# openxrlab/xrnerf

Hardware: NVIDIA B200
Metric: rays/sec (inference render, Instant-NGP lego-shaped 800x800, 65536 rays/batch) (higher is better)
Workload: dtype f16

## Files before the change

### xrnerf_b200/csrc/common.cuh

```cuda
#pragma once
#include <cuda_runtime.h>
#include <cuda_fp16.h>
#include <stdint.h>
#include <float.h>
#include "../../include/xrnerf_b200.h"

namespace xrb {

constexpr uint32_t NERF_STEPS = 1024u;
constexpr uint32_t NERF_CASCADES = 8u;
constexpr uint32_t NERF_GRIDSIZE = 128u;
constexpr uint32_t GRID_CELLS = 128u * 128u * 128u;
constexpr float NERF_MIN_OPTICAL_THICKNESS = 0.01f;
constexpr int NUM_SMS = 148;

__host__ __device__ constexpr float SQRT3() { return 1.73205080757f; }
__host__ __device__ constexpr float MIN_CONE_STEPSIZE() { return SQRT3() / NERF_STEPS; }
__host__ __device__ constexpr float MAX_CONE_STEPSIZE() { return (SQRT3() / NERF_STEPS) * (1 << (NERF_CASCADES - 1)) * NERF_STEPS / NERF_GRIDSIZE; }

void set_error(const char *msg);
int check_launch(const char *what);

#define XRB_REQUIRE(cond, msg)                                   \
    do {                                                         \
        if (!(cond)) { xrb::set_error(msg); return XRB_E_BADARG; } \
    } while (0)

struct Pcg32 {
    uint64_t state, inc;
    __host__ __device__ uint32_t next_uint() {
        uint64_t old = state;
        state = old * 0x5851f42d4c957f2dULL + inc;
        uint32_t xorshifted = (uint32_t)(((old >> 18u) ^ old) >> 27u);
        uint32_t rot = (uint32_t)(old >> 59u);
        return (xorshifted >> rot) | (xorshifted << ((~rot + 1u) & 31));
    }
    __host__ __device__ void seed(uint64_t initstate, uint64_t initseq) {
        state = 0; inc = (initseq << 1u) | 1u; next_uint(); state += initstate; next_uint();
    }
    __host__ __device__ float next_float() {
#ifdef __CUDA_ARCH__
        return __fadd_rn(__uint_as_float((next_uint() >> 9) | 0x3f800000u), -1.0f);
#else
        union { uint32_t u; float f; } x; x.u = (next_uint() >> 9) | 0x3f800000u; return x.f - 1.0f;
#endif
    }
    __host__ __device__ void advance(uint64_t delta) {
        uint64_t cur_mult = 0x5851f42d4c957f2dULL, cur_plus = inc, acc_mult = 1u, acc_plus = 0u;
        while (delta > 0) {
            if (delta & 1) { acc_mult *= cur_mult; acc_plus = acc_plus * cur_mult + cur_plus; }
            cur_plus = (cur_mult + 1) * cur_plus; cur_mult *= cur_mult; delta /= 2;
        }
        state = acc_mult * state + acc_plus;
    }
};
inline Pcg32 host_rng(uint64_t seed, int64_t n_prior_calls) {
    Pcg32 r; r.seed(seed, 1u);
    r.advance((uint64_t)n_prior_calls << 32);
    return r;
}

__host__ __device__ __forceinline__ uint32_t expand_bits(uint32_t v) {
    v = (v * 0x00010001u) & 0xFF0000FFu; v = (v * 0x00000101u) & 0x0F00F00Fu;
    v = (v * 0x00000011u) & 0xC30C30C3u; v = (v * 0x00000005u) & 0x49249249u; return v;
}
__host__ __device__ __forceinline__ uint32_t morton3D(uint32_t x, uint32_t y, uint32_t z) { return expand_bits(x) | (expand_bits(y) << 1) | (expand_bits(z) << 2); }
__host__ __device__ __forceinline__ uint32_t morton3D_invert(uint32_t x) {
    x = x & 0x49249249; x = (x | (x >> 2)) & 0xc30c30c3; x = (x | (x >> 4)) & 0x0f00f00f;
    x = (x | (x >> 8)) & 0xff0000ff; x = (x | (x >> 16)) & 0x0000ffff; return x;
}

#ifdef __CUDACC__
__device__ __forceinline__ float mul_(float a, float b) { return __fmul_rn(a, b); }
__device__ __forceinline__ float add_(float a, float b) { return __fadd_rn(a, b); }
__device__ __forceinline__ float sub_(float a, float b) { return __fsub_rn(a, b); }
__device__ __forceinline__ float div_(float a, float b) { return __fdiv_rn(a, b); }
__device__ __forceinline__ float clampf(float v, float lo, float hi) { return v < lo ? lo : (hi < v ? hi : v); }
__device__ __forceinline__ float calc_dt(float t, float cone) { return clampf(mul_(t, cone), MIN_CONE_STEPSIZE(), MAX_CONE_STEPSIZE()); }

__device__ __forceinline__ float floor_small(float p, int *ip) {
    float t = __fadd_rn(p, 12582912.0f);
    float r = __fadd_rn(t, -12582912.0f);
    int i = __float_as_int(t) - 0x4B400000;
    if (r > p) { r = __fadd_rn(r, -1.0f); i -= 1; }
    *ip = i;
    return r;
}
__device__ __forceinline__ uint32_t expand_bits7(uint32_t v) {
    v = (v | (v << 8)) & 0x0000F00Fu;
    v = (v | (v << 4)) & 0x000C30C3u;
    v = (v | (v << 2)) & 0x00249249u;
    return v;
}

__device__ __forceinline__ int frexp_exponent(float v) {
    uint32_t e = __float_as_uint(v) >> 23;
    if (e != 0) return (int)e - 126;
    if (v == 0.f) return 0;
    int r; frexpf(v, &r); return r;
}
__device__ __forceinline__ int mip_from_pos(float px, float py, float pz) {
    float m = fmaxf(fabsf(sub_(px, 0.5f)), fmaxf(fabsf(sub_(py, 0.5f)), fabsf(sub_(pz, 0.5f))));
    if (m >= 0.25f) return min((int)NERF_CASCADES - 1, (int)(__float_as_uint(m) >> 23) - 125);
    return m == 0.f ? 1 : 0;
}
__device__ __forceinline__ int mip_from_dt(float dt, float px, float py, float pz) {
    int mip = mip_from_pos(px, py, pz);
    dt = mul_(dt, (float)(2 * NERF_GRIDSIZE));
    if (dt < 1.f) return mip;
    int e = (int)(__float_as_uint(dt) >> 23) - 126;
    return min((int)NERF_CASCADES - 1, max(e, mip));
}
__device__ __forceinline__ void morton_lut_init(uint32_t *lut, int tid, int nthreads) {
    for (int v = tid; v < 128; v += nthreads) lut[v] = expand_bits7((uint32_t)v);
}
__device__ __forceinline__ uint32_t cascaded_grid_idx_at(float px, float py, float pz, uint32_t mip, const uint32_t *lut = nullptr) {
    float s = __uint_as_float((127u - mip) << 23);
    float q[3] = {px, py, pz}; uint32_t c[3];
#pragma unroll
    for (int k = 0; k < 3; ++k) {
        float v = add_(mul_(sub_(q[k], 0.5f), s), 0.5f);
        int i; floor_small(mul_(v, (float)NERF_GRIDSIZE), &i);
        c[k] = (uint32_t)min(max(i, 0), (int)NERF_GRIDSIZE - 1);
    }
    if (lut) return lut[c[0]] + (lut[c[1]] << 1) + (lut[c[2]] << 2);
    return expand_bits7(c[0]) | (expand_bits7(c[1]) << 1) | (expand_bits7(c[2]) << 2);
}
__device__ __forceinline__ bool occupied_at(float px, float py, float pz, const uint8_t *__restrict__ bitfield, uint32_t mip, const uint32_t *lut = nullptr) {
    uint32_t idx = cascaded_grid_idx_at(px, py, pz, mip, lut);
    return __ldg(bitfield + (idx >> 3) + ((GRID_CELLS * mip) >> 3)) & (1u << (idx & 7u));
}
__device__ __forceinline__ float signf_(float x) { return copysignf(1.0f, x); }
__device__ __forceinline__ float distance_to_next_voxel(const float p[3], const float d[3], const float idir[3], uint32_t res) {
    float t3[3];
#pragma unroll
    for (int k = 0; k < 3; ++k) {
        float pr = mul_((float)res, p[k]);
        int unused; float fl = floor_small(add_(add_(pr, 0.5f), mul_(0.5f, signf_(d[k]))), &unused);
        t3[k] = mul_(sub_(fl, pr), idir[k]);
    }
    float t = fminf(fminf(t3[0], t3[1]), t3[2]);
    return fmaxf(mul_(t, __uint_as_float((254u - (__float_as_uint((float)res) >> 23)) << 23)), 0.0f);
}
__device__ __forceinline__ float advance_to_next_voxel(float t, float cone, const float p[3], const float d[3], const float idir[3], uint32_t res) {
    float t_target = add_(t, distance_to_next_voxel(p, d, idir, res));
    do { t = add_(t, calc_dt(t, cone)); } while (t < t_target);
    return t;
}
__device__ __forceinline__ float aabb_ray_tmin(float lo, float hi, const float o[3], const float d[3]) {
    float tmin = div_(sub_(lo, o[0]), d[0]), tmax = div_(sub_(hi, o[0]), d[0]);
    if (tmin > tmax) { float c = tmin; tmin = tmax; tmax = c; }
    float tymin = div_(sub_(lo, o[1]), d[1]), tymax = div_(sub_(hi, o[1]), d[1]);
    if (tymin > tymax) { float c = tymin; tymin = tymax; tymax = c; }
    if (tmin > tymax || tymin > tmax) return FLT_MAX;
    if (tymin > tmin) tmin = tymin;
    if (tymax < tmax) tmax = tymax;
    float tzmin = div_(sub_(lo, o[2]), d[2]), tzmax = div_(sub_(hi, o[2]), d[2]);
    if (tzmin > tzmax) { float c = tzmin; tzmin = tzmax; tzmax = c; }
    if (tmin > tzmax || tzmin > tmax) return FLT_MAX;
    if (tzmin > tmin) tmin = tzmin;
    return tmin;
}
__device__ __forceinline__ bool aabb_contains(float lo, float hi, float x, float y, float z) {
    return x >= lo && x <= hi && y >= lo && y <= hi && z >= lo && z <= hi;
}
__device__ __forceinline__ float warp_dt(float dt) {
    const float max_stepsize = MIN_CONE_STEPSIZE() * (1 << (NERF_CASCADES - 1));
    return div_(sub_(dt, MIN_CONE_STEPSIZE()), max_stepsize - MIN_CONE_STEPSIZE());
}
__device__ __forceinline__ float unwarp_dt(float dt) {
    const float max_stepsize = MIN_CONE_STEPSIZE() * (1 << (NERF_CASCADES - 1));
    return add_(mul_(dt, max_stepsize - MIN_CONE_STEPSIZE()), MIN_CONE_STEPSIZE());
}
__device__ __forceinline__ float ray_start_t(Pcg32 rng, uint32_t i, float lo, float hi, const float o[3], const float d[3], float near_distance, float cone) {
    rng.advance((uint64_t)(i * 8u));
    float tmin = fmaxf(aabb_ray_tmin(lo, hi, o, d), near_distance);
    return add_(tmin, mul_(calc_dt(tmin, cone), rng.next_float()));
}

__device__ __forceinline__ float logistic(float x) { return 1.0f / (1.0f + expf(-x)); }
__device__ __forceinline__ float net_to_rgb(float v, int act) {
    switch (act) { case 0: return v; case 1: return v > 0.f ? v : 0.f; case 2: return logistic(v); case 3: return __expf(clampf(v, -10.f, 10.f)); }
    return 0.f;
}
__device__ __forceinline__ float net_to_density(float v, int act) {
    switch (act) { case 0: return v; case 1: return v > 0.f ? v : 0.f; case 2: return logistic(v); case 3: return __expf(v); }
    return 0.f;
}
__device__ __forceinline__ float net_to_rgb_deriv(float v, int act) {
    switch (act) { case 0: return 1.f; case 1: return v > 0.f ? 1.f : 0.f; case 2: { float s = logistic(v); return s * (1 - s); } case 3: return __expf(clampf(v, -10.f, 10.f)); }
    return 0.f;
}
__device__ __forceinline__ float net_to_density_deriv(float v, int act) {
    switch (act) { case 0: return 1.f; case 1: return v > 0.f ? 1.f : 0.f; case 2: { float s = logistic(v); return s * (1 - s); } case 3: return __expf(clampf(v, -15.f, 15.f)); }
    return 0.f;
}

__device__ __forceinline__ uint32_t warp_incl_scan_u32(uint32_t v, int lane) {
#pragma unroll
    for (int o = 1; o < 32; o <<= 1) { uint32_t n = __shfl_up_sync(0xffffffffu, v, o); if (lane >= o) v += n; }
    return v;
}
#endif

}
```

### xrnerf_b200/csrc/ngp_field.cuh

```cuda
#pragma once
#include "common.cuh"

namespace xrb {

constexpr int MAX_LEVELS = 16;
struct HashGridDev {
    uint32_t offset[MAX_LEVELS + 1];
    float scale[MAX_LEVELS];
    uint32_t res[MAX_LEVELS];
    int n_levels;
    uint32_t hashed_mask;
    uint32_t packed_mask;
    uint32_t cell_off[MAX_LEVELS];
};

inline int64_t hashgrid_build(const xrb_ngp_config *cfg, HashGridDev *g) {
    g->n_levels = cfg->n_levels; g->hashed_mask = 0;
    const float log2_pls = log2f(cfg->per_level_scale);
    uint32_t off = 0;
    for (int l = 0; l < cfg->n_levels; ++l) {
        float scale = exp2f(l * log2_pls) * (float)cfg->base_resolution - 1.0f;
        uint32_t res = (uint32_t)ceilf(scale) + 1;
        uint64_t cube = (uint64_t)res * res * res; uint32_t maxp = 0xffffffffu / 2;
        uint32_t p = cube > maxp ? maxp : (uint32_t)cube;
        p = (p + 7u) / 8u * 8u;
        uint32_t cap = 1u << cfg->log2_hashmap_size; if (p > cap) p = cap;
        if (cube > p) g->hashed_mask |= 1u << l;
        g->offset[l] = off; g->scale[l] = scale; g->res[l] = res; off += p;
    }
    g->offset[cfg->n_levels] = off;
    g->packed_mask = 0;
    for (int l = 0; l < MAX_LEVELS; ++l) g->cell_off[l] = 0;
    return (int64_t)off * cfg->n_features;
}
inline size_t cell_image_layout(HashGridDev *g, int n_packed) {
    size_t rec = 0; g->packed_mask = 0;
    for (int l = 0; l < g->n_levels && l < n_packed; ++l) {
        g->cell_off[l] = (uint32_t)rec; g->packed_mask |= 1u << l;
        rec += (size_t)g->res[l] * g->res[l] * g->res[l];
    }
    return rec * 32;
}
constexpr int MAX_PACKED_LEVELS = 13;
__host__ __device__ inline int64_t mlp_num_params(int in_w, int width, int n_hidden, int out_pad) { return (int64_t)width * in_w + (int64_t)(n_hidden - 1) * width * width + (int64_t)out_pad * width; }

inline int check_cfg(const xrb_ngp_config *cfg) {
    if (!cfg) { set_error("ngp config is null"); return XRB_E_BADARG; }
    if (cfg->n_levels != 16 || cfg->n_features != 2 || cfg->width != 64 || cfg->density_hidden < 1 || cfg->density_hidden > 4 || cfg->color_hidden < 1 || cfg->color_hidden > 4 ||
        cfg->log2_hashmap_size < 8 || cfg->log2_hashmap_size > 24 || cfg->base_resolution < 1) {
        set_error("ngp config unsupported: need n_levels=16, n_features=2, n_neurons=64, 1..4 hidden layers");
        return XRB_E_UNSUPPORTED;
    }
    return XRB_OK;
}

int table_setup(const xrb_ngp_config *cfg, const xrb_ngp_table *t, HashGridDev *g, const char *who);
struct HashGridDev;
int launch_field_ps(const xrb_ngp_config *cfg, const HashGridDev &g, const xrb_ngp_table *tab, const void *image, const float *pts, int pts_stride, const float *dirs, int dirs_stride, int n,
                    const int32_t *n_dev, float *raw, cudaStream_t s);
int launch_field(const xrb_ngp_config *cfg, const xrb_ngp_table *table, const void *dens, const void *color, const void *image, const float *pts, int pts_stride, const float *dirs,
                 int dirs_stride, int n, const int32_t *n_dev, float *out, int impl, bool density_only, cudaStream_t s);

#ifdef __CUDACC__
__device__ __forceinline__ float round_h(float x) { return __half2float(__float2half_rn(x)); }

__device__ __forceinline__ uint32_t grid_index(uint32_t x, uint32_t y, uint32_t z, uint32_t hashmap_size, uint32_t res) {
    if ((uint64_t)res * res * res > hashmap_size) {
        uint32_t h = x ^ (y * 2654435761u) ^ (z * 805459861u);
        return h & (hashmap_size - 1);
    }
    uint32_t index = x + y * res + z * res * res;
    return index >= hashmap_size ? index - hashmap_size : index;
}

struct __align__(32) Cell32 { uint32_t v[8]; };
__device__ __forceinline__ Cell32 ldg_cell(const void *p) {
    Cell32 r;
    asm volatile("ld.global.nc.v8.b32 {%0,%1,%2,%3,%4,%5,%6,%7}, [%8];"
                 : "=r"(r.v[0]), "=r"(r.v[1]), "=r"(r.v[2]), "=r"(r.v[3]), "=r"(r.v[4]), "=r"(r.v[5]), "=r"(r.v[6]), "=r"(r.v[7]) : "l"(p));
    return r;
}
__device__ __forceinline__ __half2 as_h2(uint32_t u) { return *reinterpret_cast<__half2 *>(&u); }

enum { GATHER_RUNTIME = 0, GATHER_PACKED = 1, GATHER_HASHED = 2, GATHER_DENSE = 3 };
template <int NP> __host__ __device__ constexpr int plan_mode(int l) { return NP == 0 ? GATHER_RUNTIME : (l < NP ? GATHER_PACKED : GATHER_HASHED); }
inline bool plan_valid(const HashGridDev &g, int np) {
    if (np <= 0 || np > g.n_levels) return false;
    const uint32_t all = g.n_levels >= 32 ? 0xffffffffu : ((1u << g.n_levels) - 1u), packed = (1u << np) - 1u;
    return g.packed_mask == packed && ((g.hashed_mask | packed) & all) == all;
}

__device__ __forceinline__ float2 hash_level(const __half2 *__restrict__ table, const uint8_t *__restrict__ cells, const HashGridDev &g, int l, float x, float y, float z,
                                             const int MODE = GATHER_RUNTIME) {
    const uint32_t off = g.offset[l], hs = g.offset[l + 1] - off, res = g.res[l];
    const float sc = g.scale[l];
    float px = __fmaf_rn(sc, x, 0.5f), py = __fmaf_rn(sc, y, 0.5f), pz = __fmaf_rn(sc, z, 0.5f);
    int ix_, iy_, iz_;
    float fx = floor_small(px, &ix_), fy = floor_small(py, &iy_), fz = floor_small(pz, &iz_);
    const uint32_t gx = (uint32_t)ix_, gy = (uint32_t)iy_, gz = (uint32_t)iz_;
    fx = px - fx; fy = py - fy; fz = pz - fz;
    __half2 v[8];
    const bool is_packed = MODE == GATHER_PACKED || (MODE == GATHER_RUNTIME && ((g.packed_mask >> l) & 1u));
    const bool is_hashed = MODE == GATHER_HASHED || (MODE == GATHER_RUNTIME && ((g.hashed_mask >> l) & 1u));
    if (is_packed) {
        const uint32_t rm1 = res - 1u, cx = min(gx, rm1), cy = min(gy, rm1), cz = min(gz, rm1);
        const Cell32 r = ldg_cell(cells + ((size_t)(g.cell_off[l] + cx + res * (cy + res * cz)) << 5));
#pragma unroll
        for (int c = 0; c < 8; ++c) v[c] = as_h2(r.v[c]);
    } else if (is_hashed) {
        const __half2 *tl = table + off;
        asm volatile("" : "+l"(tl));
        const uint32_t mask = hs - 1u;
        const uint32_t hy0 = gy * 2654435761u, hy1 = hy0 + 2654435761u, hz0 = gz * 805459861u, hz1 = hz0 + 805459861u;
        const uint32_t a00 = hy0 ^ hz0, a10 = hy1 ^ hz0, a01 = hy0 ^ hz1, a11 = hy1 ^ hz1, gx1 = gx + 1u;
        const uint32_t i0 = (gx ^ a00) & mask, i1 = (gx ^ a10) & mask, i2 = (gx ^ a01) & mask, i3 = (gx ^ a11) & mask;
        const uint2 w0 = __ldg(reinterpret_cast<const uint2 *>(tl + (i0 & ~1u))), w1 = __ldg(reinterpret_cast<const uint2 *>(tl + (i1 & ~1u))),
                    w2 = __ldg(reinterpret_cast<const uint2 *>(tl + (i2 & ~1u))), w3 = __ldg(reinterpret_cast<const uint2 *>(tl + (i3 & ~1u)));
        uint32_t n0 = 0, n1 = 0, n2 = 0, n3 = 0;
        const bool odd = gx & 1u;
        if (odd) {
            n0 = __ldg(reinterpret_cast<const uint32_t *>(tl + ((gx1 ^ a00) & mask))); n1 = __ldg(reinterpret_cast<const uint32_t *>(tl + ((gx1 ^ a10) & mask)));
            n2 = __ldg(reinterpret_cast<const uint32_t *>(tl + ((gx1 ^ a01) & mask))); n3 = __ldg(reinterpret_cast<const uint32_t *>(tl + ((gx1 ^ a11) & mask)));
        }
        const uint32_t e0 = (i0 & 1u) ? w0.y : w0.x, o0 = (i0 & 1u) ? w0.x : w0.y, e1 = (i1 & 1u) ? w1.y : w1.x, o1 = (i1 & 1u) ? w1.x : w1.y;
        const uint32_t e2 = (i2 & 1u) ? w2.y : w2.x, o2 = (i2 & 1u) ? w2.x : w2.y, e3 = (i3 & 1u) ? w3.y : w3.x, o3 = (i3 & 1u) ? w3.x : w3.y;
        v[0] = as_h2(e0); v[1] = as_h2(odd ? n0 : o0);
        v[2] = as_h2(e1); v[3] = as_h2(odd ? n1 : o1);
        v[4] = as_h2(e2); v[5] = as_h2(odd ? n2 : o2);
        v[6] = as_h2(e3); v[7] = as_h2(odd ? n3 : o3);
    } else {
        const __half2 *tl = table + off;
        asm volatile("" : "+l"(tl));
        const uint32_t sy = res, sz = res * res, b = gx + gy * sy + gz * sz;
#pragma unroll
        for (int c = 0; c < 8; ++c) {
            uint32_t idx = b + (c & 1) + ((c >> 1) & 1) * sy + ((c >> 2) & 1) * sz;
            idx = idx >= hs ? idx - hs : idx;
            v[c] = __ldg(tl + idx);
        }
    }
    const float ux = 1.f - fx, uy = 1.f - fy, uz = 1.f - fz;
    float2 acc = make_float2(0.f, 0.f);
#pragma unroll
    for (int c = 0; c < 8; ++c) {
        float w = ((c & 1) ? fx : ux) * ((c & 2) ? fy : uy) * ((c & 4) ? fz : uz);
        float2 f = __half22float2(v[c]);
        acc.x += w * f.x; acc.y += w * f.y;
    }
    return acc;
}

__device__ __forceinline__ void sh4(float dx01, float dy01, float dz01, float *out) {
    float x = dx01 * 2.f - 1.f, y = dy01 * 2.f - 1.f, z = dz01 * 2.f - 1.f;
    float xy = x * y, xz = x * z, yz = y * z, x2 = x * x, y2 = y * y, z2 = z * z;
    out[0] = 0.28209479177387814f;
    out[1] = -0.48860251190291987f * y;
    out[2] = 0.48860251190291987f * z;
    out[3] = -0.48860251190291987f * x;
    out[4] = 1.0925484305920792f * xy;
    out[5] = -1.0925484305920792f * yz;
    out[6] = 0.94617469575755997f * z2 - 0.31539156525251999f;
    out[7] = -1.0925484305920792f * xz;
    out[8] = 0.54627421529603959f * x2 - 0.54627421529603959f * y2;
    out[9] = 0.59004358992664352f * y * (-3.0f * x2 + y2);
    out[10] = 2.8906114426405538f * xy * z;
    out[11] = 0.45704579946446572f * y * (1.0f - 5.0f * z2);
    out[12] = 0.3731763325901154f * z * (5.0f * z2 - 3.0f);
    out[13] = 0.45704579946446572f * x * (1.0f - 5.0f * z2);
    out[14] = 1.4453057213202769f * z * (x2 - y2);
    out[15] = 0.59004358992664352f * x * (-x2 + 3.0f * y2);
}

__host__ __device__ __forceinline__ uint32_t sw128_offset(uint32_t row, uint32_t chunk16) {
    return (row >> 3) * 1024u + (row & 7u) * 128u + ((chunk16 ^ (row & 7u)) << 4);
}
struct WeightImageLayout {
    uint32_t d_in, d_hid[3], d_out, c_in, c_hid[3], c_out, total;
};
__host__ __device__ inline WeightImageLayout weight_image_layout(int density_hidden, int color_hidden) {
    WeightImageLayout L{}; uint32_t o = 0;
    L.d_in = o; o += 64 * 128;
    for (int k = 0; k < density_hidden - 1; ++k) { L.d_hid[k] = o; o += 64 * 128; }
    L.d_out = o; o += 16 * 128;
    L.c_in = o; o += 64 * 128;
    for (int k = 0; k < color_hidden - 1; ++k) { L.c_hid[k] = o; o += 64 * 128; }
    L.c_out = o; o += 16 * 128;
    L.total = o;
    return L;
}
#endif

}
```

### xrnerf_b200/csrc/ngp_fused.cu

```cuda
#include "tc_field.cuh"
#include <stdio.h>
#include <stdlib.h>

namespace xrb {

constexpr uint32_t FR_ROW_BYTES = 80;
constexpr uint32_t FR_SLOT_BYTES = 128 * FR_ROW_BYTES;
constexpr uint32_t FR_TCAP = 64;
constexpr int FR_MAX_WG = 2;

struct FusedParams {
    HashGridDev g;
    const __half2 *table; const uint8_t *cells; int np; const void *weight_image; uint32_t image_bytes; int density_hidden, color_hidden;
    const uint8_t *bitfield; const float *rays_o; const float *rays_d; int n_rays;
    float lo, hi, near_distance, cone; Pcg32 rng;
    float bg[3]; int rgb_act, dens_act;
    float *rgb_out; float *alpha_out; int32_t *n_samples_out;
    float *tscratch;
    uint32_t *sched;
    unsigned long long *dbg_out;
    int dbg;
    int field_only; const float *pts; int pts_stride; const float *dirs; int dirs_stride; int n_samples; const int32_t *n_dev; float4 *raw_out;
};

template <int FR_N_WG, int N_PROD, int N_SLOTS>
struct FusedCtl {
    uint64_t full[N_SLOTS];
    uint64_t mail[N_PROD][2];
    uint64_t mma[FR_N_WG], wbar;
    uint32_t rounds_done[N_SLOTS];
    uint32_t owner[N_SLOTS][4];
    uint32_t issued_bcast[FR_N_WG];
    uint32_t tmem_slot, ticket, closed, done, prod_done;
    uint32_t morton[128];
};
template <int FR_N_WG, int N_PROD, int N_SLOTS>
__host__ __device__ inline size_t fused_smem_bytes(uint32_t image_bytes) {
    return 1024 + image_bytes + (size_t)FR_N_WG * 16384 + (size_t)N_SLOTS * FR_SLOT_BYTES + (size_t)N_PROD * 1024 + sizeof(FusedCtl<FR_N_WG, N_PROD, N_SLOTS>) + 64;
}

__device__ __forceinline__ void spin_until_ge(volatile uint32_t *p, uint32_t v) {
    while (*p < v) __nanosleep(20);
}

template <int FR_N_WG, int N_PROD, int N_SLOTS>
__global__ void __launch_bounds__((4 * FR_N_WG + N_PROD) * 32, 3 - FR_N_WG) ngp_render_fused_kernel(const __grid_constant__ FusedParams P) {
    extern __shared__ uint8_t dyn_smem[];
    using Ctl = FusedCtl<FR_N_WG, N_PROD, N_SLOTS>;
    uint8_t *base = (uint8_t *)(((uintptr_t)dyn_smem + 1023) & ~(uintptr_t)1023);
    uint8_t *W = base, *A = W + P.image_bytes, *slots = A + (size_t)FR_N_WG * 16384, *mailbox = slots + (size_t)N_SLOTS * FR_SLOT_BYTES;
    Ctl *ctl = (Ctl *)(mailbox + (size_t)N_PROD * 1024);
    const uint32_t warp = threadIdx.x >> 5, lane = threadIdx.x & 31;
    if ((P.dbg & 8) && threadIdx.x == 0) {
        unsigned long long t0; uint32_t smid;
        asm volatile("mov.u64 %0, %%globaltimer;" : "=l"(t0)); asm volatile("mov.u32 %0, %%smid;" : "=r"(smid));
        P.dbg_out[16 * blockIdx.x] = t0; P.dbg_out[16 * blockIdx.x + 2] = smid; for (int k = 3; k < 16; ++k) P.dbg_out[16 * blockIdx.x + k] = 0;
    }

    if (threadIdx.x == 0) {
        for (int k = 0; k < N_SLOTS; ++k) { tc::mbar_init(ctl->full + k, 4); ctl->rounds_done[k] = 0; }
        for (int k = 0; k < N_PROD; ++k) { tc::mbar_init(&ctl->mail[k][0], 32); tc::mbar_init(&ctl->mail[k][1], 32); }
        for (int k = 0; k < FR_N_WG; ++k) { tc::mbar_init(ctl->mma + k, 1); ctl->issued_bcast[k] = 0; }
        tc::mbar_init(&ctl->wbar, 1);
        ctl->ticket = 0; ctl->closed = 0; ctl->done = 0; ctl->prod_done = 0;
        tc::fence_mbar_init();
        tc::mbar_expect_tx(&ctl->wbar, P.image_bytes);
        tc::tma_bulk_g2s(W, P.weight_image, P.image_bytes, &ctl->wbar);
    }
    if (warp == 1) tc::tmem_alloc<64 * FR_N_WG>(&ctl->tmem_slot);
    morton_lut_init(ctl->morton, threadIdx.x, blockDim.x);
    tc::tc_fence_before_sync();
    __syncthreads();
    tc::tc_fence_after_sync();
    const uint32_t tmem_base = ctl->tmem_slot;

    if (warp < 4 * FR_N_WG) {
        TcWarpgroup c;
        c.wg = warp >> 2; c.row = threadIdx.x & 127;
        c.A = A + (size_t)c.wg * 16384; c.W = W; c.mbar = ctl->mma + c.wg; c.tmem = tmem_base + c.wg * 64; c.phase = 0;
        const WeightImageLayout L = weight_image_layout(P.density_hidden, P.color_hidden);
        const bool timed = (P.dbg & 8) && c.wg == 0;
        tc::mbar_wait(&ctl->wbar, 0);
        long long fc[5] = {0, 0, 0, 0, 0}, ck = 0; (void)ck; (void)timed;
#ifdef XRB_FUSED_TIMERS
#define FTICK(k) do { if (timed) { long long n_ = clock64(); fc[k] += n_ - ck; ck = n_; } } while (0)
#else
#define FTICK(k) do { } while (0)
#endif
        for (uint32_t X = c.wg;; X += FR_N_WG) {
            const uint32_t s = X % N_SLOTS, r = X / N_SLOTS;
            FTICK(4);
            if (c.row == 0) {
                volatile uint32_t *tk = &ctl->ticket; volatile uint32_t *dn = &ctl->done; volatile uint32_t *cl = &ctl->closed;
                while (*cl != X) __nanosleep(20);
                uint32_t issued = 0;
                while (true) {
                    if (*tk > 4 * X) { issued = 1; break; }
                    if (*dn) { if (*tk > 4 * X) issued = 1; break; }
                    __nanosleep(20);
                }
                if (issued) {
                    while (true) {
                        uint32_t cur = *tk;
                        if (cur >= 4 * (X + 1)) { issued = 4; break; }
                        if (atomicCAS(&ctl->ticket, cur, 4 * (X + 1)) == cur) { issued = cur - 4 * X; break; }
                    }
                    for (uint32_t k = issued; k < 4; ++k) tc::mbar_arrive(ctl->full + s);
                }
                ctl->issued_bcast[c.wg] = issued;
                __threadfence_block();
                *cl = X + 1;
            }
            tc::named_bar_sync(3 + c.wg, 128);
            const uint32_t issued = *(volatile uint32_t *)&ctl->issued_bcast[c.wg];
            FTICK(0);
            if (issued == 0) { if (timed && c.row == 0) { P.dbg_out[16 * blockIdx.x + 3] = X; for (int k = 0; k < 5; ++k) P.dbg_out[16 * blockIdx.x + 4 + k] = (unsigned long long)fc[k]; } break; }
            tc::mbar_wait(ctl->full + s, r & 1);
            FTICK(1);
            const uint8_t *rowp = slots + (size_t)s * FR_SLOT_BYTES + (size_t)c.row * FR_ROW_BYTES;
            const uint4 f0 = *reinterpret_cast<const uint4 *>(rowp), f1 = *reinterpret_cast<const uint4 *>(rowp + 16), f2 = *reinterpret_cast<const uint4 *>(rowp + 32),
                        f3 = *reinterpret_cast<const uint4 *>(rowp + 48);
            const float4 dir = *reinterpret_cast<const float4 *>(rowp + 64);
            const uint32_t sub = c.row >> 5;
            const uint32_t own = ctl->owner[s][sub];
            a_store_chunk(c, 0, f0); a_store_chunk(c, 1, f1); a_store_chunk(c, 2, f2); a_store_chunk(c, 3, f3);
            tc::named_bar_sync(3 + c.wg, 128);
            if (c.row == 0) { __threadfence_block(); *(volatile uint32_t *)&ctl->rounds_done[s] = r + 1; }
            FTICK(2);
            float4 raw = make_float4(0.f, 0.f, 0.f, 0.f);
            if (!(P.dbg & 2)) {
                float dout[16];
                tc_density_from_a(c, L, P.density_hidden, dout);
                raw = tc_color_from_density(c, L, P.color_hidden, dout, dir.x, dir.y, dir.z);
            }
            FTICK(3);
            if (sub < issued) {
                *reinterpret_cast<float4 *>(mailbox + (size_t)own * 512 + (c.row & 31) * 16) = raw;
                tc::mbar_arrive(&ctl->mail[own >> 1][own & 1]);
            }
        }
    } else {
        const uint32_t pw = warp - 4 * FR_N_WG;
        float *tb = P.tscratch + ((size_t)blockIdx.x * N_PROD + pw) * 32 * FR_TCAP;
        const float diag = sub_(P.hi, P.lo);
        uint32_t n_submitted = 0;
        long long pc[7] = {0, 0, 0, 0, 0, 0, 0}, ck = 0; (void)ck;
#ifdef XRB_FUSED_TIMERS
#define PTICK(k) do { if (P.dbg & 8) { long long n_ = clock64(); pc[k] += n_ - ck; ck = n_; } } while (0)
#else
#define PTICK(k) do { } while (0)
#endif
        auto submit_chunk = [&](float x, float y, float z, float wd0, float wd1, float wd2) {
            uint32_t tk = 0;
            if (lane == 0) tk = atomicAdd(&ctl->ticket, 1u);
            tk = __shfl_sync(0xffffffffu, tk, 0);
            const uint32_t X = tk >> 2, sub = tk & 3, s = X % N_SLOTS, r = X / N_SLOTS;
            if (lane == 0) { spin_until_ge(&ctl->rounds_done[s], r); __threadfence_block(); ctl->owner[s][sub] = (pw << 1) | (n_submitted & 1); }
            __syncwarp();
            PTICK(5);
            uint8_t *rowp = slots + (size_t)s * FR_SLOT_BYTES + (size_t)(sub * 32 + lane) * FR_ROW_BYTES;
            *reinterpret_cast<float4 *>(rowp + 64) = make_float4(wd0, wd1, wd2, 0.f);
            if (P.dbg & 1) {
                for (int l = 0; l < 16; ++l) *reinterpret_cast<uint32_t *>(rowp + 4 * l) = pack_h2(x, y);
            } else if (P.np > 0) {
#pragma unroll 1
                for (int l = 0; l < P.np; ++l) {
                    const float2 f = hash_level(P.table, P.cells, P.g, l, x, y, z, GATHER_PACKED);
                    *reinterpret_cast<uint32_t *>(rowp + 4 * l) = pack_h2(f.x, f.y);
                }
#pragma unroll 1
                for (int l = P.np; l < 16; ++l) {
                    const float2 f = hash_level(P.table, P.cells, P.g, l, x, y, z, GATHER_HASHED);
                    *reinterpret_cast<uint32_t *>(rowp + 4 * l) = pack_h2(f.x, f.y);
                }
            } else {
#pragma unroll 1
                for (int l = 0; l < 16; ++l) {
                    const float2 f = hash_level(P.table, P.cells, P.g, l, x, y, z, GATHER_RUNTIME);
                    *reinterpret_cast<uint32_t *>(rowp + 4 * l) = pack_h2(f.x, f.y);
                }
            }
            __syncwarp();
            if (lane == 0) tc::mbar_arrive(ctl->full + s);
        };
        if (P.field_only) {
            int n = P.n_samples;
            if (P.n_dev) n = min(n, max(*P.n_dev, 0));
            bool pending = false, prev_valid = false; int prev_q = 0;
            const uint32_t n_pw = gridDim.x * N_PROD;
            for (uint32_t chunk = blockIdx.x * N_PROD + pw;; chunk += n_pw) {
                const bool have_chunk = (uint64_t)chunk * 32 < (uint64_t)n;
                int q = 0; bool valid = false;
                if (have_chunk) {
                    q = (int)(chunk * 32u + lane); valid = q < n;
                    float x = 0.5f, y = 0.5f, z = 0.5f, wd0 = 0.5f, wd1 = 0.5f, wd2 = 0.5f;
                    if (valid) {
                        const float *c = P.pts + (size_t)q * P.pts_stride, *d = P.dirs + (size_t)q * P.dirs_stride;
                        x = __ldg(c); y = __ldg(c + 1); z = __ldg(c + 2); wd0 = __ldg(d); wd1 = __ldg(d + 1); wd2 = __ldg(d + 2);
                    }
                    submit_chunk(x, y, z, wd0, wd1, wd2);
                }
                if (pending) {
                    const uint32_t kprev = n_submitted - 1;
                    if (lane == 0) tc::mbar_wait(&ctl->mail[pw][kprev & 1], (kprev >> 1) & 1);
                    __syncwarp();
                    const float4 raw = *reinterpret_cast<const float4 *>(mailbox + (size_t)((pw << 1) | (kprev & 1)) * 512 + lane * 16);
                    if (prev_valid) P.raw_out[prev_q] = raw;
                    pending = false;
                }
                if (!have_chunk) break;
                ++n_submitted; pending = true; prev_q = q; prev_valid = valid;
            }
        } else
        for (;;) {
            PTICK(6);
            uint32_t grp = 0;
            if (lane == 0) grp = atomicAdd(P.sched, 1u);
            grp = __shfl_sync(0xffffffffu, grp, 0);
            if ((uint64_t)grp * 32 >= (uint64_t)P.n_rays) break;
            const uint32_t ray = grp * 32 + lane;
            bool alive = ray < (uint32_t)P.n_rays;
            float t = 0.f; uint32_t nsteps = 0;
            if (alive) {
                const float o[3] = {__ldg(P.rays_o + 3 * (size_t)ray), __ldg(P.rays_o + 3 * (size_t)ray + 1), __ldg(P.rays_o + 3 * (size_t)ray + 2)};
                const float d[3] = {__ldg(P.rays_d + 3 * (size_t)ray), __ldg(P.rays_d + 3 * (size_t)ray + 1), __ldg(P.rays_d + 3 * (size_t)ray + 2)};
                t = ray_start_t(P.rng, ray, P.lo, P.hi, o, d, P.near_distance, P.cone);
            }
            float T = 1.f, ax = 0.f, ay = 0.f, az = 0.f;
            bool any_alive;
            do {
                uint32_t m = 0;
                if (alive && (P.dbg & 4)) {
                    float *tl = tb + (size_t)lane * FR_TCAP;
                    for (; m < 11; ++m) { tl[m] = t; t += 0.01f; }
                    nsteps = 11; alive = false;
                }
                if (alive) {
                    const float o[3] = {__ldg(P.rays_o + 3 * (size_t)ray), __ldg(P.rays_o + 3 * (size_t)ray + 1), __ldg(P.rays_o + 3 * (size_t)ray + 2)};
                    const float d[3] = {__ldg(P.rays_d + 3 * (size_t)ray), __ldg(P.rays_d + 3 * (size_t)ray + 1), __ldg(P.rays_d + 3 * (size_t)ray + 2)};
                    const float idir[3] = {div_(1.0f, d[0]), div_(1.0f, d[1]), div_(1.0f, d[2])};
                    float *tl = tb + (size_t)lane * FR_TCAP;
                    while (true) {
                        float p[3] = {add_(o[0], mul_(t, d[0])), add_(o[1], mul_(t, d[1])), add_(o[2], mul_(t, d[2]))};
                        if (!(aabb_contains(P.lo, P.hi, p[0], p[1], p[2]) && nsteps < NERF_STEPS)) { alive = false; break; }
                        float dt = calc_dt(t, P.cone);
                        uint32_t mip = (uint32_t)mip_from_dt(dt, p[0], p[1], p[2]);
                        if (occupied_at(p[0], p[1], p[2], P.bitfield, mip, ctl->morton)) {
                            tl[m] = t; ++m; ++nsteps; t = add_(t, dt);
                            if (m == FR_TCAP) break;
                        } else {
                            t = advance_to_next_voxel(t, P.cone, p, d, idir, NERF_GRIDSIZE >> mip);
                        }
                    }
                }
                __syncwarp();
                PTICK(0);
                any_alive = __any_sync(0xffffffffu, alive);
                const uint32_t incl = warp_incl_scan_u32(m, lane);
                const uint32_t rbase = incl - m, total = __shfl_sync(0xffffffffu, incl, 31);

                bool pending = false; uint32_t pend_key = 0; float pend_dt = 0.f;
                for (uint32_t q0 = 0; q0 < total || pending; q0 += 32) {
                    const bool have_chunk = q0 < total;
                    float dtc = 0.f; uint32_t key = 32u + lane;
                    PTICK(6);
                    if (have_chunk) {
                        const uint32_t q = q0 + lane;
                        const bool valid = q < total;
                        uint32_t j = 0;
#pragma unroll
                        for (uint32_t step = 16; step >= 1; step >>= 1) {
                            const uint32_t cand = j + step;
                            const uint32_t b = __shfl_sync(0xffffffffu, rbase, cand & 31);
                            if (cand < 32 && b <= q) j = cand;
                        }
                        const uint32_t bj = __shfl_sync(0xffffffffu, rbase, j);
                        float x = 0.5f, y = 0.5f, z = 0.5f, wd0 = 0.5f, wd1 = 0.5f, wd2 = 0.5f;
                        if (valid) {
                            const float tt = *(volatile float *)(tb + (size_t)j * FR_TCAP + (q - bj));
                            const size_t rj = (size_t)grp * 32 + j;
                            const float oj0 = __ldg(P.rays_o + 3 * rj), oj1 = __ldg(P.rays_o + 3 * rj + 1), oj2 = __ldg(P.rays_o + 3 * rj + 2);
                            const float dj0 = __ldg(P.rays_d + 3 * rj), dj1 = __ldg(P.rays_d + 3 * rj + 1), dj2 = __ldg(P.rays_d + 3 * rj + 2);
                            x = div_(sub_(add_(oj0, mul_(tt, dj0)), P.lo), diag); y = div_(sub_(add_(oj1, mul_(tt, dj1)), P.lo), diag); z = div_(sub_(add_(oj2, mul_(tt, dj2)), P.lo), diag);
                            wd0 = mul_(add_(dj0, 1.0f), 0.5f); wd1 = mul_(add_(dj1, 1.0f), 0.5f); wd2 = mul_(add_(dj2, 1.0f), 0.5f);
                            dtc = unwarp_dt(warp_dt(calc_dt(tt, P.cone)));
                            key = j;
                        }
#ifdef XRB_FUSED_TIMERS
                        if (P.dbg & 8) { if (__float_as_uint(x + y + z + dtc) == 0x7fc12345u) pc[6] += 1; }
#endif
                        PTICK(1);
                        submit_chunk(x, y, z, wd0, wd1, wd2);
                        PTICK(2);
                    }
                    if (pending) {
                        const uint32_t kprev = n_submitted - 1;
                        if (lane == 0) tc::mbar_wait(&ctl->mail[pw][kprev & 1], (kprev >> 1) & 1);
                        __syncwarp();
                        PTICK(3);
                        const float4 raw = *reinterpret_cast<const float4 *>(mailbox + (size_t)((pw << 1) | (kprev & 1)) * 512 + lane * 16);
                        float alpha = 0.f, sx = 0.f, sy = 0.f, sz = 0.f;
                        if (pend_key < 32) {
                            const float density = net_to_density(raw.w, P.dens_act);
                            alpha = 1.f - __expf(-density * pend_dt);
                            sx = alpha * net_to_rgb(raw.x, P.rgb_act); sy = alpha * net_to_rgb(raw.y, P.rgb_act); sz = alpha * net_to_rgb(raw.z, P.rgb_act);
                        }
                        float pr = 1.f - alpha;
                        const uint32_t prev_key = __shfl_up_sync(0xffffffffu, pend_key, 1);
                        const uint32_t heads = __ballot_sync(0xffffffffu, lane == 0 || pend_key != prev_key);
                        const int seg_start = 31 - __clz(heads & (0xffffffffu >> (31 - lane)));
#pragma unroll
                        for (int off = 1; off < 32; off <<= 1) {
                            const float np = __shfl_up_sync(0xffffffffu, pr, off), nx = __shfl_up_sync(0xffffffffu, sx, off), ny = __shfl_up_sync(0xffffffffu, sy, off),
                                        nz = __shfl_up_sync(0xffffffffu, sz, off);
                            if ((int)lane - off >= seg_start) { sx = nx + np * sx; sy = ny + np * sy; sz = nz + np * sz; pr = np * pr; }
                        }
                        const uint32_t pq0 = q0 - 32;
                        const uint32_t lo_q = max(rbase, pq0), hi_q = min(rbase + m, q0);
                        const uint32_t tail = (hi_q - 1 - pq0) & 31;
                        const float gp = __shfl_sync(0xffffffffu, pr, tail), gx = __shfl_sync(0xffffffffu, sx, tail), gy = __shfl_sync(0xffffffffu, sy, tail),
                                    gz = __shfl_sync(0xffffffffu, sz, tail);
                        if (hi_q > lo_q) { ax += T * gx; ay += T * gy; az += T * gz; T *= gp; }
                        pending = false;
                        PTICK(4);
                    }
                    if (have_chunk) { ++n_submitted; pending = true; pend_key = key; pend_dt = dtc; }
                }
            } while (any_alive);
            if (ray < (uint32_t)P.n_rays) {
                P.rgb_out[3 * (size_t)ray] = ax + T * P.bg[0]; P.rgb_out[3 * (size_t)ray + 1] = ay + T * P.bg[1]; P.rgb_out[3 * (size_t)ray + 2] = az + T * P.bg[2];
                P.alpha_out[ray] = 1.f - T;
                if (P.n_samples_out) P.n_samples_out[ray] = (int32_t)nsteps;
            }
        }
        if ((P.dbg & 8) && lane == 0) { for (int k = 0; k < 7; ++k) atomicAdd(P.dbg_out + 16 * blockIdx.x + 9 + k, (unsigned long long)pc[k]); }
        if (lane == 0) {
            __threadfence_block();
            if (atomicAdd(&ctl->prod_done, 1u) == N_PROD - 1) *(volatile uint32_t *)&ctl->done = 1u;
        }
    }
    tc::tc_fence_before_sync();
    __syncthreads();
    if (warp == 1) tc::tmem_dealloc<64 * FR_N_WG>(tmem_base);
    if ((P.dbg & 8) && threadIdx.x == 0) { unsigned long long t1; asm volatile("mov.u64 %0, %%globaltimer;" : "=l"(t1)); P.dbg_out[16 * blockIdx.x + 1] = t1; }
    if (threadIdx.x == 0 && !P.field_only) {
        __threadfence();
        if (atomicAdd(P.sched + 1, 1u) == gridDim.x - 1) { P.sched[0] = 0; P.sched[1] = 0; __threadfence(); }
    }
}

constexpr int FUSED_MAX_PROD_PER_SM = 24;
static int fused_variant() { static int v = -1; if (v < 0) { const char *e = getenv("XRB_FUSED_VARIANT"); v = e ? atoi(e) : 0; if (v != 0 && v != 1) v = 0; } return v; }

int launch_field_ps(const xrb_ngp_config *cfg, const HashGridDev &g, const xrb_ngp_table *tab, const void *image, const float *pts, int pts_stride, const float *dirs, int dirs_stride, int n,
                    const int32_t *n_dev, float *raw, cudaStream_t s) {
    FusedParams P{};
    P.g = g;
    P.table = (const __half2 *)tab->table_fp16; P.cells = (const uint8_t *)tab->cell_image; P.np = plan_valid(P.g, tab->n_packed_levels) ? tab->n_packed_levels : 0;
    P.weight_image = image; P.image_bytes = weight_image_layout(cfg->density_hidden, cfg->color_hidden).total;
    P.density_hidden = cfg->density_hidden; P.color_hidden = cfg->color_hidden;
    P.field_only = 1; P.pts = pts; P.pts_stride = pts_stride; P.dirs = dirs; P.dirs_stride = dirs_stride; P.n_samples = n; P.n_dev = n_dev; P.raw_out = (float4 *)raw;
    { static const int dbg = getenv("XRB_FUSED_DBG") ? atoi(getenv("XRB_FUSED_DBG")) : 0; P.dbg = dbg & 3; }
    int dev = 0, sms = NUM_SMS; cudaGetDevice(&dev); cudaDeviceGetAttribute(&sms, cudaDevAttrMultiProcessorCount, dev);
    auto k = ngp_render_fused_kernel<2, 16, 5>;
    const size_t smem = fused_smem_bytes<2, 16, 5>(P.image_bytes);
    cudaFuncSetAttribute(k, cudaFuncAttributeMaxDynamicSharedMemorySize, (int)smem);
    const int64_t n_chunks = ((int64_t)n + 31) / 32;
    int grid = sms; if (n_chunks < (int64_t)grid * 16) grid = (int)((n_chunks + 15) / 16); if (grid < 1) grid = 1;
    k<<<grid, (4 * 2 + 16) * 32, smem, s>>>(P);
    return check_launch("ngp_mlp_forward (producer/consumer)");
}

}

using namespace xrb;

extern "C" {

size_t xrb_ngp_render_fused_workspace(void) {
    int dev = 0, sms = NUM_SMS; cudaGetDevice(&dev); if (cudaDeviceGetAttribute(&sms, cudaDevAttrMultiProcessorCount, dev) != cudaSuccess) { cudaGetLastError(); sms = NUM_SMS; }
    return 256 + (size_t)sms * FUSED_MAX_PROD_PER_SM * 32 * FR_TCAP * sizeof(float) + (size_t)sms * 2 * 128;
}

int xrb_ngp_render_fused(const xrb_ngp_config *cfg, const xrb_ngp_table *table, const void *weight_image, const uint8_t *bitfield, const float *rays_o, const float *rays_d, int n_rays,
                         float aabb0, float aabb1, float near_distance, float cone_angle, uint64_t seed, int64_t n_prior_calls, const float *bg3_host, int rgb_act, int dens_act,
                         float *rgb_out, float *alpha_out, int32_t *n_samples_out, void *workspace, void *stream) {
    int e = check_cfg(cfg); if (e) return e;
    XRB_REQUIRE(n_rays >= 0, "ngp_render_fused: bad size");
    if (n_rays == 0) return XRB_OK;
    XRB_REQUIRE(table && weight_image && bitfield && rays_o && rays_d && bg3_host && rgb_out && alpha_out && workspace, "ngp_render_fused: null pointer");
    XRB_REQUIRE(((uintptr_t)workspace & 255) == 0 && ((uintptr_t)weight_image & 15) == 0, "ngp_render_fused: workspace must be 256-byte aligned, weight image 16-byte aligned");
    FusedParams P;
    e = table_setup(cfg, table, &P.g, "ngp_render_fused"); if (e) return e;
    P.table = (const __half2 *)table->table_fp16; P.cells = (const uint8_t *)table->cell_image; P.np = plan_valid(P.g, table->n_packed_levels) ? table->n_packed_levels : 0;
    P.weight_image = weight_image; P.image_bytes = weight_image_layout(cfg->density_hidden, cfg->color_hidden).total;
    P.density_hidden = cfg->density_hidden; P.color_hidden = cfg->color_hidden;
    P.bitfield = bitfield; P.rays_o = rays_o; P.rays_d = rays_d; P.n_rays = n_rays;
    P.lo = aabb0; P.hi = aabb1; P.near_distance = near_distance; P.cone = cone_angle; P.rng = host_rng(seed, n_prior_calls);
    P.bg[0] = bg3_host[0]; P.bg[1] = bg3_host[1]; P.bg[2] = bg3_host[2]; P.rgb_act = rgb_act; P.dens_act = dens_act;
    P.rgb_out = rgb_out; P.alpha_out = alpha_out; P.n_samples_out = n_samples_out;
    { static const int dbg = getenv("XRB_FUSED_DBG") ? atoi(getenv("XRB_FUSED_DBG")) : 0; P.dbg = dbg; }
    int dev = 0, sms = NUM_SMS; cudaGetDevice(&dev); cudaDeviceGetAttribute(&sms, cudaDevAttrMultiProcessorCount, dev);
    P.sched = (uint32_t *)workspace; P.tscratch = (float *)((uint8_t *)workspace + 256);
    P.dbg_out = (unsigned long long *)((uint8_t *)workspace + 256 + (size_t)sms * FUSED_MAX_PROD_PER_SM * 32 * FR_TCAP * sizeof(float));
    const int64_t n_groups = ((int64_t)n_rays + 31) / 32;
    P.field_only = 0; P.pts = nullptr; P.dirs = nullptr; P.pts_stride = P.dirs_stride = 0; P.n_samples = 0; P.n_dev = nullptr; P.raw_out = nullptr;
#define XRB_LAUNCH_FUSED(NWG, NP, NS)                                                                                                                  \
    do {                                                                                                                                               \
        auto k = ngp_render_fused_kernel<NWG, NP, NS>;                                                                                                 \
        const size_t smem = fused_smem_bytes<NWG, NP, NS>(P.image_bytes);                                                                              \
        cudaFuncSetAttribute(k, cudaFuncAttributeMaxDynamicSharedMemorySize, (int)smem);    \
        int grid = sms * (3 - NWG); if (n_groups < grid) grid = (int)n_groups;                                                                         \
        k<<<grid, (4 * NWG + NP) * 32, smem, (cudaStream_t)stream>>>(P);                                                                               \
    } while (0)
    if (fused_variant() == 1) XRB_LAUNCH_FUSED(1, 8, 3); else XRB_LAUNCH_FUSED(2, 16, 5);
#undef XRB_LAUNCH_FUSED
    return check_launch("ngp_render_fused");
}

}
```

### xrnerf_b200/csrc/ngp_mlp.cu

```cuda
#include "tc_field.cuh"
#include <stdio.h>
#include <stdlib.h>

namespace xrb {

__global__ void __launch_bounds__(256) cast_f32_to_f16_kernel(const float *__restrict__ src, __half *__restrict__ dst, int64_t n) {
    int64_t i = ((int64_t)blockIdx.x * blockDim.x + threadIdx.x) * 4;
    const int64_t stride = (int64_t)gridDim.x * blockDim.x * 4;
    for (; i + 3 < n; i += stride) {
        float4 v = *reinterpret_cast<const float4 *>(src + i);
        __half2 a = __floats2half2_rn(v.x, v.y), b = __floats2half2_rn(v.z, v.w);
        uint2 o; o.x = *reinterpret_cast<uint32_t *>(&a); o.y = *reinterpret_cast<uint32_t *>(&b);
        *reinterpret_cast<uint2 *>(dst + i) = o;
    }
    if (blockIdx.x == 0 && threadIdx.x < 4) { int64_t t = (n & ~(int64_t)3) + threadIdx.x; if (t < n) dst[t] = __float2half_rn(src[t]); }
}

__global__ void pack_weights_kernel(const float *__restrict__ dens, const float *__restrict__ color, uint8_t *__restrict__ image, int density_hidden, int color_hidden) {
    const WeightImageLayout L = weight_image_layout(density_hidden, color_hidden);
    const int n_mats = density_hidden + 1 + color_hidden + 1;
    for (int m = blockIdx.x; m < n_mats; m += gridDim.x) {
        const bool is_color = m > density_hidden;
        const int li = is_color ? m - (density_hidden + 1) : m;
        const int n_hidden = is_color ? color_hidden : density_hidden;
        const float *params = is_color ? color : dens;
        const int K = li == 0 ? 32 : 64, N = li == n_hidden ? 16 : 64;
        size_t poff = 0;
        for (int q = 0; q < li; ++q) poff += (size_t)64 * (q == 0 ? 32 : 64);
        const float *Wm = params + poff;
        uint32_t ioff = is_color ? (li == 0 ? L.c_in : (li == n_hidden ? L.c_out : L.c_hid[li - 1])) : (li == 0 ? L.d_in : (li == n_hidden ? L.d_out : L.d_hid[li - 1]));
        for (int t = threadIdx.x; t < N * 8; t += blockDim.x) {
            int row = t >> 3, chunk = t & 7;
            __half h[8];
#pragma unroll
            for (int e = 0; e < 8; ++e) { int k = chunk * 8 + e; h[e] = k < K ? __float2half_rn(Wm[(size_t)row * K + k]) : __float2half_rn(0.f); }
            *reinterpret_cast<uint4 *>(image + ioff + sw128_offset(row, chunk)) = *reinterpret_cast<uint4 *>(h);
        }
    }
}

__global__ void __launch_bounds__(256) cell_image_build_kernel(HashGridDev g, const __half2 *__restrict__ table, uint32_t *__restrict__ image, int n_packed, uint64_t n_words) {
    for (uint64_t t = (uint64_t)blockIdx.x * blockDim.x + threadIdx.x; t < n_words; t += (uint64_t)gridDim.x * blockDim.x) {
        const uint32_t rec = (uint32_t)(t >> 3), c = (uint32_t)t & 7u;
        int l = 0;
#pragma unroll
        for (int k = 1; k < MAX_PACKED_LEVELS; ++k) if (k < n_packed && rec >= g.cell_off[k]) l = k;
        const uint32_t res = g.res[l], cell = rec - g.cell_off[l];
        const uint32_t gx = cell % res, gy = (cell / res) % res, gz = cell / (res * res);
        const uint32_t hs = g.offset[l + 1] - g.offset[l];
        const uint32_t idx = grid_index(gx + (c & 1u), gy + ((c >> 1) & 1u), gz + ((c >> 2) & 1u), hs, res);
        image[t] = reinterpret_cast<const uint32_t *>(table)[g.offset[l] + idx];
    }
}

__global__ void __launch_bounds__(256) hashgrid_forward_kernel(HashGridDev g, const __half2 *__restrict__ table, const uint8_t *__restrict__ cells, const float *__restrict__ x,
                                                               int x_stride, int n, __half2 *__restrict__ enc) {
    int64_t t = (int64_t)blockIdx.x * blockDim.x + threadIdx.x;
    int64_t i = t >> 4; int l = (int)(t & 15);
    if (i >= n) return;
    const float *p = x + (size_t)i * x_stride;
    float2 f = hash_level(table, cells, g, l, p[0], p[1], p[2]);
    enc[(size_t)i * 16 + l] = __floats2half2_rn(f.x, f.y);
}
__global__ void __launch_bounds__(256) sh4_forward_kernel(const float *__restrict__ dirs, int stride, int n, __half *__restrict__ out) {
    int i = blockIdx.x * blockDim.x + threadIdx.x;
    if (i >= n) return;
    const float *d = dirs + (size_t)i * stride;
    float s[16]; sh4(d[0], d[1], d[2], s);
    __half h[16];
#pragma unroll
    for (int k = 0; k < 16; ++k) h[k] = __float2half_rn(s[k]);
    uint4 *o = reinterpret_cast<uint4 *>(out + (size_t)i * 16);
    o[0] = reinterpret_cast<uint4 *>(h)[0]; o[1] = reinterpret_cast<uint4 *>(h)[1];
}

template <int IN, int OUT, bool RELU>
__device__ __forceinline__ void simt_layer(const __half *__restrict__ W, const float *x, float *y) {
#pragma unroll
    for (int o = 0; o < OUT; ++o) {
        float s = 0.f;
        const __half2 *w2 = reinterpret_cast<const __half2 *>(W + (size_t)o * IN);
#pragma unroll
        for (int k = 0; k < IN / 2; ++k) { float2 w = __half22float2(w2[k]); s = fmaf(w.x, x[2 * k], s); s = fmaf(w.y, x[2 * k + 1], s); }
        y[o] = round_h(RELU ? fmaxf(s, 0.f) : s);
    }
}
__device__ __forceinline__ void simt_net(const __half *__restrict__ P, int n_hidden, const float *x32, float *out16) {
    float a[64], b[64];
    simt_layer<32, 64, true>(P, x32, a); P += 64 * 32;
    for (int h = 0; h < n_hidden - 1; ++h) {
        simt_layer<64, 64, true>(P, a, b); P += 64 * 64;
#pragma unroll
        for (int k = 0; k < 64; ++k) a[k] = b[k];
    }
    simt_layer<64, 16, false>(P, a, out16);
}

template <bool DENSITY_ONLY>
__global__ void __launch_bounds__(128) ngp_field_simt_kernel(HashGridDev g, const __half2 *__restrict__ table, const uint8_t *__restrict__ cells, const __half *__restrict__ dens_p, const __half *__restrict__ color_p,
                                                             int density_hidden, int color_hidden, const float *__restrict__ pts, int pts_stride, const float *__restrict__ dirs,
                                                             int dirs_stride, int n, const int32_t *__restrict__ n_dev, float *__restrict__ out) {
    extern __shared__ __half s_w[];
    if (n_dev) n = min(n, max(*n_dev, 0));
    const int nd = (int)mlp_num_params(32, 64, density_hidden, 16), nc = DENSITY_ONLY ? 0 : (int)mlp_num_params(32, 64, color_hidden, 16);
    for (int k = threadIdx.x; k < nd; k += blockDim.x) s_w[k] = dens_p[k];
    for (int k = threadIdx.x; k < nc; k += blockDim.x) s_w[nd + k] = color_p[k];
    __syncthreads();
    for (int i = blockIdx.x * blockDim.x + threadIdx.x; i < n; i += gridDim.x * blockDim.x) {
        const float *p = pts + (size_t)i * pts_stride;
        float enc[32];
#pragma unroll
        for (int l = 0; l < 16; ++l) { float2 f = hash_level(table, cells, g, l, p[0], p[1], p[2]); enc[2 * l] = round_h(f.x); enc[2 * l + 1] = round_h(f.y); }
        float dout[16];
        simt_net(s_w, density_hidden, enc, dout);
        if (DENSITY_ONLY) { out[i] = dout[0]; continue; }
        const float *d = dirs + (size_t)i * dirs_stride;
        float cin[32], sh[16];
        sh4(d[0], d[1], d[2], sh);
#pragma unroll
        for (int k = 0; k < 15; ++k) cin[k] = dout[k + 1];
#pragma unroll
        for (int k = 0; k < 16; ++k) cin[15 + k] = round_h(sh[k]);
        cin[31] = 1.0f;
        float cout[16];
        simt_net(s_w + nd, color_hidden, cin, cout);
        reinterpret_cast<float4 *>(out)[i] = make_float4(cout[0], cout[1], cout[2], dout[0]);
    }
}

__global__ void __launch_bounds__(128) mlp_forward_simt_kernel(const __half *__restrict__ params, const __half *__restrict__ x, int n, int n_hidden, __half *__restrict__ y) {
    extern __shared__ __half s_w[];
    const int np = (int)mlp_num_params(32, 64, n_hidden, 16);
    for (int k = threadIdx.x; k < np; k += blockDim.x) s_w[k] = params[k];
    __syncthreads();
    for (int i = blockIdx.x * blockDim.x + threadIdx.x; i < n; i += gridDim.x * blockDim.x) {
        float xin[32], out[16];
#pragma unroll
        for (int k = 0; k < 32; ++k) xin[k] = __half2float(x[(size_t)i * 32 + k]);
        simt_net(s_w, n_hidden, xin, out);
#pragma unroll
        for (int k = 0; k < 16; ++k) y[(size_t)i * 16 + k] = __float2half_rn(out[k]);
    }
}

template <bool DENSITY_ONLY, int NWG, int MAXREG, int NP>
__global__ void __launch_bounds__(128 * NWG, NWG == 2 ? 2 : 1) __maxnreg__(MAXREG)
ngp_field_tc_kernel(HashGridDev g, const __half2 *__restrict__ table, const uint8_t *__restrict__ cells, const void *__restrict__ weight_image, uint32_t image_bytes, int density_hidden,
                    int color_hidden, const float *__restrict__ pts, int pts_stride, const float *__restrict__ dirs, int dirs_stride, int n, const int32_t *__restrict__ n_dev,
                    float *__restrict__ out, int dbg) {
    extern __shared__ uint8_t dyn_smem[];
    if (n_dev) n = min(n, max(*n_dev, 0));
    constexpr uint32_t TMEM_COLS = NWG <= 2 ? 128 : (NWG <= 4 ? 256 : 512);
    TcWarpgroup c = tc_cta_setup<NWG, TMEM_COLS>(dyn_smem, weight_image, image_bytes);
    const uint32_t tmem_base = c.tmem - c.wg * 64;
    const WeightImageLayout L = weight_image_layout(density_hidden, color_hidden);
    const int n_tiles = (n + 127) / 128;
    if (!(dbg & 7)) {
        const int stride = gridDim.x * NWG;
        int tile = blockIdx.x * NWG + c.wg;
        if (tile < n_tiles) {
            uint32_t e[16];
            float dx = 0.5f, dy = 0.5f, dz = 0.5f;
            {
                const int i = tile * 128 + c.row;
                float x = 0.5f, y = 0.5f, z = 0.5f;
                if (i < n) {
                    const float *p = pts + (size_t)i * pts_stride; x = p[0]; y = p[1]; z = p[2];
                    if (!DENSITY_ONLY) { const float *d = dirs + (size_t)i * dirs_stride; dx = d[0]; dy = d[1]; dz = d[2]; }
                }
                tc_gather_levels<NP, 0, 16>(table, cells, g, x, y, z, e);
            }
            for (; tile < n_tiles; tile += stride) {
                const int i = tile * 128 + c.row, in = i + stride * 128;
                const bool has_next = tile + stride < n_tiles;
                float xn = 0.5f, yn = 0.5f, zn = 0.5f, dxn = 0.5f, dyn = 0.5f, dzn = 0.5f;
                if (has_next && in < n) {
                    const float *p = pts + (size_t)in * pts_stride; xn = p[0]; yn = p[1]; zn = p[2];
                    if (!DENSITY_ONLY) { const float *d = dirs + (size_t)in * dirs_stride; dxn = d[0]; dyn = d[1]; dzn = d[2]; }
                }
                uint32_t en[16];
                const float4 raw = tc_field_gather_ahead<NP, DENSITY_ONLY>(c, L, density_hidden, color_hidden, table, cells, g, e, dx, dy, dz, has_next, xn, yn, zn, en);
                if (i < n) { if (DENSITY_ONLY) out[i] = raw.x; else reinterpret_cast<float4 *>(out)[i] = raw; }
#pragma unroll
                for (int k = 0; k < 16; ++k) e[k] = en[k];
                dx = dxn; dy = dyn; dz = dzn;
            }
        }
        tc_cta_teardown<TMEM_COLS>(tmem_base);
        return;
    }
    for (int tile = blockIdx.x * NWG + c.wg; tile < n_tiles; tile += gridDim.x * NWG) {
        const int i = tile * 128 + c.row;
        const bool valid = i < n;
        float x = 0.5f, y = 0.5f, z = 0.5f, dx = 0.5f, dy = 0.5f, dz = 0.5f;
        if (valid) {
            const float *p = pts + (size_t)i * pts_stride; x = p[0]; y = p[1]; z = p[2];
            if (!DENSITY_ONLY) { const float *d = dirs + (size_t)i * dirs_stride; dx = d[0]; dy = d[1]; dz = d[2]; }
        }
        float dout[16];
        if (dbg & 1) {
#pragma unroll
            for (int q = 0; q < 4; ++q) a_store_chunk(c, q, make_uint4(pack_h2(x, y), pack_h2(z, x), pack_h2(y, z), pack_h2(x, z)));
            if (dbg & 2) { for (int k = 0; k < 16; ++k) dout[k] = x; } else tc_density_from_a(c, L, density_hidden, dout);
        } else if (dbg & 2) {
            float acc = 0.f;
#pragma unroll
            for (int l = 0; l < 16; ++l) { float2 f = hash_level(table, cells, g, l, x, y, z, plan_mode<NP>(l)); acc += f.x + f.y; }
            for (int k = 0; k < 16; ++k) dout[k] = acc;
        } else {
            tc_density<NP>(c, L, density_hidden, table, cells, g, x, y, z, dout);
        }
        if (DENSITY_ONLY) {
            if (valid) out[i] = dout[0];
        } else {
            float4 raw = (dbg & 2) ? make_float4(dout[0], dout[1], dout[2], dout[3]) : tc_color_from_density(c, L, color_hidden, dout, dx, dy, dz);
            if (valid) reinterpret_cast<float4 *>(out)[i] = raw;
        }
    }
    tc_cta_teardown<TMEM_COLS>(tmem_base);
}

static int persistent_grid(const void *kernel, int block, size_t smem, int work_ctas, int min_per_sm = 1) {
    int per_sm = 1;
    cudaError_t oe = cudaOccupancyMaxActiveBlocksPerMultiprocessor(&per_sm, kernel, block, smem);
    if (getenv("XRB_DEBUG")) fprintf(stderr, "[xrb] occupancy query: err=%d per_sm=%d block=%d smem=%zu\n", (int)oe, per_sm, block, smem);
    if (oe != cudaSuccess) cudaGetLastError();
    if (per_sm < min_per_sm) per_sm = min_per_sm;
    int dev = 0, sms = NUM_SMS; cudaGetDevice(&dev); cudaDeviceGetAttribute(&sms, cudaDevAttrMultiProcessorCount, dev);
    int g = sms * per_sm;
    return work_ctas < g ? (work_ctas > 0 ? work_ctas : 1) : g;
}

}

using namespace xrb;

extern "C" {

int64_t xrb_tcnn_hashgrid_num_params(const xrb_ngp_config *cfg) { if (check_cfg(cfg)) return -1; HashGridDev g; return hashgrid_build(cfg, &g); }
int64_t xrb_tcnn_density_num_params(const xrb_ngp_config *cfg) { if (check_cfg(cfg)) return -1; return mlp_num_params(32, 64, cfg->density_hidden, 16); }
int64_t xrb_tcnn_color_num_params(const xrb_ngp_config *cfg) { if (check_cfg(cfg)) return -1; return mlp_num_params(32, 64, cfg->color_hidden, 16); }
int xrb_tcnn_hashgrid_layout(const xrb_ngp_config *cfg, uint32_t *offsets_host, float *scales_host, uint32_t *res_host) {
    int e = check_cfg(cfg); if (e) return e;
    HashGridDev g; hashgrid_build(cfg, &g);
    for (int l = 0; l <= cfg->n_levels; ++l) if (offsets_host) offsets_host[l] = g.offset[l];
    for (int l = 0; l < cfg->n_levels; ++l) { if (scales_host) scales_host[l] = g.scale[l]; if (res_host) res_host[l] = g.res[l]; }
    return XRB_OK;
}

int xrb_tcnn_cast_params(const float *src, void *dst_fp16, int64_t n, void *stream) {
    XRB_REQUIRE(n >= 0, "cast_params: negative size");
    if (n == 0) return XRB_OK;
    XRB_REQUIRE(src && dst_fp16, "cast_params: null pointer");
    XRB_REQUIRE(((uintptr_t)src & 15) == 0 && ((uintptr_t)dst_fp16 & 7) == 0, "cast_params: misaligned");
    int64_t blocks = (n / 4 + 255) / 256; if (blocks > NUM_SMS * 16) blocks = NUM_SMS * 16; if (blocks < 1) blocks = 1;
    cast_f32_to_f16_kernel<<<(int)blocks, 256, 0, (cudaStream_t)stream>>>(src, (__half *)dst_fp16, n);
    return check_launch("cast_params");
}

size_t xrb_ngp_weight_image_bytes(const xrb_ngp_config *cfg) { if (check_cfg(cfg)) return 0; return weight_image_layout(cfg->density_hidden, cfg->color_hidden).total; }

int xrb_ngp_pack_weights(const xrb_ngp_config *cfg, const float *density_params, const float *color_params, void *image, void *stream) {
    int e = check_cfg(cfg); if (e) return e;
    XRB_REQUIRE(density_params && color_params && image, "pack_weights: null pointer");
    XRB_REQUIRE(((uintptr_t)image & 15) == 0, "pack_weights: image must be 16-byte aligned");
    pack_weights_kernel<<<cfg->density_hidden + cfg->color_hidden + 2, 256, 0, (cudaStream_t)stream>>>(density_params, color_params, (uint8_t *)image, cfg->density_hidden, cfg->color_hidden);
    return check_launch("pack_weights");
}

size_t xrb_ngp_cell_image_bytes(const xrb_ngp_config *cfg, int n_packed_levels) {
    if (check_cfg(cfg) || n_packed_levels <= 0) return 0;
    if (n_packed_levels > MAX_PACKED_LEVELS) n_packed_levels = MAX_PACKED_LEVELS;
    HashGridDev g; hashgrid_build(cfg, &g);
    return cell_image_layout(&g, n_packed_levels);
}

int xrb_ngp_build_cell_image(const xrb_ngp_config *cfg, const void *table_fp16, int n_packed_levels, void *cell_image, void *stream) {
    int e = check_cfg(cfg); if (e) return e;
    XRB_REQUIRE(n_packed_levels >= 0 && n_packed_levels <= MAX_PACKED_LEVELS, "build_cell_image: n_packed_levels must be 0..13");
    if (n_packed_levels == 0) return XRB_OK;
    XRB_REQUIRE(table_fp16 && cell_image, "build_cell_image: null pointer");
    XRB_REQUIRE(((uintptr_t)cell_image & 31) == 0 && ((uintptr_t)table_fp16 & 15) == 0, "build_cell_image: cell image must be 32-byte, table 16-byte aligned");
    HashGridDev g; hashgrid_build(cfg, &g);
    const uint64_t n_words = cell_image_layout(&g, n_packed_levels) / 4;
    uint64_t blocks = (n_words + 255) / 256; if (blocks > (uint64_t)NUM_SMS * 32) blocks = (uint64_t)NUM_SMS * 32;
    cell_image_build_kernel<<<(unsigned)blocks, 256, 0, (cudaStream_t)stream>>>(g, (const __half2 *)table_fp16, (uint32_t *)cell_image, n_packed_levels, n_words);
    return check_launch("build_cell_image");
}

}
namespace xrb {
int table_setup(const xrb_ngp_config *cfg, const xrb_ngp_table *t, HashGridDev *g, const char *who) {
    if (!t || !t->table_fp16) { set_error("null hash table"); return XRB_E_BADARG; }
    if (((uintptr_t)t->table_fp16 & 15) != 0) { set_error("hash table must be 16-byte aligned"); return XRB_E_BADARG; }
    hashgrid_build(cfg, g);
    if (t->n_packed_levels < 0 || t->n_packed_levels > MAX_PACKED_LEVELS) { set_error("n_packed_levels must be 0..13"); return XRB_E_BADARG; }
    if (t->n_packed_levels > 0) {
        if (!t->cell_image || ((uintptr_t)t->cell_image & 31) != 0) { set_error("cell image missing or not 32-byte aligned"); return XRB_E_BADARG; }
        cell_image_layout(g, t->n_packed_levels);
    }
    (void)who;
    return XRB_OK;
}
}
extern "C" {

int xrb_tcnn_hashgrid_forward(const xrb_ngp_config *cfg, const xrb_ngp_table *table, const float *x, int x_stride, int n, void *enc_fp16, void *stream) {
    int e = check_cfg(cfg); if (e) return e;
    XRB_REQUIRE(n >= 0 && x_stride >= 3, "hashgrid_forward: bad size");
    if (n == 0) return XRB_OK;
    XRB_REQUIRE(table && x && enc_fp16, "hashgrid_forward: null pointer");
    HashGridDev g; e = table_setup(cfg, table, &g, "hashgrid_forward"); if (e) return e;
    int64_t threads = (int64_t)n * 16;
    hashgrid_forward_kernel<<<(unsigned)((threads + 255) / 256), 256, 0, (cudaStream_t)stream>>>(g, (const __half2 *)table->table_fp16, (const uint8_t *)table->cell_image, x, x_stride, n,
                                                                                                 (__half2 *)enc_fp16);
    return check_launch("hashgrid_forward");
}

int xrb_tcnn_sh4_forward(const float *dirs, int dir_stride, int n, void *out_fp16, void *stream) {
    XRB_REQUIRE(n >= 0 && dir_stride >= 3, "sh4_forward: bad size");
    if (n == 0) return XRB_OK;
    XRB_REQUIRE(dirs && out_fp16, "sh4_forward: null pointer");
    sh4_forward_kernel<<<(n + 255) / 256, 256, 0, (cudaStream_t)stream>>>(dirs, dir_stride, n, (__half *)out_fp16);
    return check_launch("sh4_forward");
}

int xrb_tcnn_mlp_forward(const void *params_fp16, const void *x_fp16, int n, int in_w, int width, int n_hidden, void *y_fp16, void *stream) {
    XRB_REQUIRE(n >= 0, "mlp_forward: negative size");
    if (in_w != 32 || width != 64 || n_hidden < 1 || n_hidden > 4) { set_error("mlp_forward: only in=32 (padded), width=64, 1..4 hidden layers"); return XRB_E_UNSUPPORTED; }
    if (n == 0) return XRB_OK;
    XRB_REQUIRE(params_fp16 && x_fp16 && y_fp16, "mlp_forward: null pointer");
    size_t smem = mlp_num_params(32, 64, n_hidden, 16) * sizeof(__half);
    if (smem > 48 * 1024) cudaFuncSetAttribute(mlp_forward_simt_kernel, cudaFuncAttributeMaxDynamicSharedMemorySize, (int)smem);
    int grid = persistent_grid((const void *)mlp_forward_simt_kernel, 128, smem, (n + 127) / 128);
    mlp_forward_simt_kernel<<<grid, 128, smem, (cudaStream_t)stream>>>((const __half *)params_fp16, (const __half *)x_fp16, n, n_hidden, (__half *)y_fp16);
    return check_launch("mlp_forward");
}

}
namespace xrb {
int launch_field(const xrb_ngp_config *cfg, const xrb_ngp_table *tab, const void *dens, const void *color, const void *image, const float *pts, int pts_stride, const float *dirs,
                 int dirs_stride, int n, const int32_t *n_dev, float *out, int impl, bool density_only, cudaStream_t s) {
    HashGridDev g; int e = table_setup(cfg, tab, &g, "field"); if (e) return e;
    const void *table = tab->table_fp16; const uint8_t *cells = (const uint8_t *)tab->cell_image;
    if (impl == 0) {
        size_t smem = (mlp_num_params(32, 64, cfg->density_hidden, 16) + (density_only ? 0 : mlp_num_params(32, 64, cfg->color_hidden, 16))) * sizeof(__half);
        const void *k = density_only ? (const void *)ngp_field_simt_kernel<true> : (const void *)ngp_field_simt_kernel<false>;
        if (smem > 48 * 1024) cudaFuncSetAttribute(k, cudaFuncAttributeMaxDynamicSharedMemorySize, (int)smem);
        int grid = persistent_grid(k, 128, smem, (n + 127) / 128);
        if (density_only)
            ngp_field_simt_kernel<true><<<grid, 128, smem, s>>>(g, (const __half2 *)table, cells, (const __half *)dens, (const __half *)color, cfg->density_hidden, cfg->color_hidden, pts, pts_stride,
                                                                dirs, dirs_stride, n, n_dev, out);
        else
            ngp_field_simt_kernel<false><<<grid, 128, smem, s>>>(g, (const __half2 *)table, cells, (const __half *)dens, (const __half *)color, cfg->density_hidden, cfg->color_hidden, pts, pts_stride,
                                                                 dirs, dirs_stride, n, n_dev, out);
    } else {
        uint32_t image_bytes = weight_image_layout(cfg->density_hidden, cfg->color_hidden).total;
        static const int env_shape = getenv("XRB_TC_SHAPE") ? atoi(getenv("XRB_TC_SHAPE")) : -1;
        const int shape = env_shape >= 0 ? env_shape : 0;
        static const int dbg = getenv("XRB_FIELD_DBG") ? atoi(getenv("XRB_FIELD_DBG")) : 0;
        if (shape == 4 && !density_only && (((uintptr_t)out) & 15) == 0) return launch_field_ps(cfg, g, tab, image, pts, pts_stride, dirs, dirs_stride, n, n_dev, out, s);
        const int npl = tab->n_packed_levels;
        const int np = (plan_valid(g, npl) && (npl == 6 || npl == 7)) ? npl : 0;
        int n_tiles = (n + 127) / 128;
#define XRB_LAUNCH_TC(D, NWG, R, NP)                                                                                                                \
    do {                                                                                                                                            \
        auto k = ngp_field_tc_kernel<D, NWG, R, NP>;                                                                                                \
        const size_t smem = tc_cta_smem_bytes<NWG>(image_bytes);                                                                                    \
        cudaFuncSetAttribute(k, cudaFuncAttributeMaxDynamicSharedMemorySize, (int)smem);                                                            \
        int grid = persistent_grid((const void *)k, 128 * NWG, smem, (n_tiles + NWG - 1) / NWG, NWG == 2 ? 2 : 1);                                  \
        k<<<grid, 128 * NWG, smem, s>>>(g, (const __half2 *)table, cells, image, image_bytes, cfg->density_hidden, cfg->color_hidden, pts, pts_stride, dirs, dirs_stride, n, n_dev, out, dbg); \
    } while (0)
#define XRB_LAUNCH_TC_NP(D, NWG, R)                                                                                                                 \
    do {                                                                                                                                            \
        if (np == 6) XRB_LAUNCH_TC(D, NWG, R, 6); else if (np == 7) XRB_LAUNCH_TC(D, NWG, R, 7); else XRB_LAUNCH_TC(D, NWG, R, 0);                   \
    } while (0)
#define XRB_LAUNCH_TC_SHAPE(D)                                                                                                                      \
    do {                                                                                                                                            \
        if (shape == 1) XRB_LAUNCH_TC_NP(D, 2, 128); else if (shape == 2) XRB_LAUNCH_TC_NP(D, 6, 80); else if (shape == 3) XRB_LAUNCH_TC_NP(D, 8, 64); else XRB_LAUNCH_TC_NP(D, 2, 96); \
    } while (0)
        if (density_only) XRB_LAUNCH_TC_SHAPE(true); else XRB_LAUNCH_TC_SHAPE(false);
#undef XRB_LAUNCH_TC_SHAPE
#undef XRB_LAUNCH_TC_NP
#undef XRB_LAUNCH_TC
    }
    return check_launch(density_only ? "ngp_density_forward" : "ngp_mlp_forward");
}
}
extern "C" {

int xrb_ngp_mlp_forward(const xrb_ngp_config *cfg, const xrb_ngp_table *table, const void *density_fp16, const void *color_fp16, const void *weight_image, const float *pts, int pts_stride,
                        const float *dirs, int dirs_stride, int n, const int32_t *n_rows_dev, float *raw, int impl, void *stream) {
    int e = check_cfg(cfg); if (e) return e;
    XRB_REQUIRE(n >= 0 && pts_stride >= 3 && dirs_stride >= 3, "ngp_mlp_forward: bad size");
    if (n == 0) return XRB_OK;
    XRB_REQUIRE(table && pts && dirs && raw, "ngp_mlp_forward: null pointer");
    XRB_REQUIRE(((uintptr_t)raw & 15) == 0, "ngp_mlp_forward: raw must be 16-byte aligned");
    XRB_REQUIRE(impl == 0 ? (density_fp16 && color_fp16) : (weight_image != nullptr), "ngp_mlp_forward: missing weights for the requested impl");
    return launch_field(cfg, table, density_fp16, color_fp16, weight_image, pts, pts_stride, dirs, dirs_stride, n, n_rows_dev, raw, impl, false, (cudaStream_t)stream);
}

int xrb_ngp_density_forward(const xrb_ngp_config *cfg, const xrb_ngp_table *table, const void *density_fp16, const void *weight_image, const float *pts, int pts_stride, int n, float *density,
                            int impl, void *stream) {
    int e = check_cfg(cfg); if (e) return e;
    XRB_REQUIRE(n >= 0 && pts_stride >= 3, "ngp_density_forward: bad size");
    if (n == 0) return XRB_OK;
    XRB_REQUIRE(table && pts && density, "ngp_density_forward: null pointer");
    XRB_REQUIRE(impl == 0 ? (density_fp16 != nullptr) : (weight_image != nullptr), "ngp_density_forward: missing weights for the requested impl");
    return launch_field(cfg, table, density_fp16, nullptr, weight_image, pts, pts_stride, nullptr, 3, n, nullptr, density, impl, true, (cudaStream_t)stream);
}

}
```

### xrnerf_b200/csrc/ngp_render.cu

```cuda
#include "ngp_field.cuh"

extern "C" {

size_t xrb_ngp_render_workspace(int n_rays, int max_samples) {
    size_t a = (xrb_rm_rays_sampler_workspace(n_rays) + 255) & ~(size_t)255;
    return a + (size_t)max_samples * (7 + 4) * sizeof(float) + (size_t)n_rays * sizeof(int32_t) + 256;
}

int xrb_ngp_render(const xrb_ngp_config *cfg, const xrb_ngp_table *table, const void *weight_image, const uint8_t *bitfield, const float *rays_o, const float *rays_d, int n_rays,
                   int max_samples, float aabb0, float aabb1, float near_distance, float cone_angle, uint64_t seed, int64_t n_prior_calls, const float *bg3_host, int rgb_act,
                   int dens_act, float *rgb_out, float *alpha_out, int32_t *numsteps, int32_t *counters, void *workspace, void *ev_before_field, void *ev_after_field, void *stream) {
    int e = xrb::check_cfg(cfg); if (e) return e;
    XRB_REQUIRE(n_rays >= 0 && max_samples > 0, "ngp_render: bad size");
    if (n_rays == 0) return XRB_OK;
    XRB_REQUIRE(table && weight_image && bitfield && rays_o && rays_d && bg3_host && rgb_out && alpha_out && numsteps && counters && workspace, "ngp_render: null pointer");
    cudaStream_t s = (cudaStream_t)stream;
    uint8_t *ws = (uint8_t *)workspace;
    size_t a = (xrb_rm_rays_sampler_workspace(n_rays) + 255) & ~(size_t)255;
    float *coords = (float *)(ws + a);
    float *raw = coords + (size_t)max_samples * 7;
    int32_t *rays_index = (int32_t *)(raw + (size_t)max_samples * 4);
    cudaMemsetAsync(counters, 0, 2 * sizeof(int32_t), s);
    e = xrb_rm_rays_sampler(rays_o, rays_d, bitfield, nullptr, nullptr, nullptr, n_rays, max_samples, aabb0, aabb1, near_distance, cone_angle, seed, n_prior_calls, coords, rays_index,
                            numsteps, counters, ws, stream);
    if (e) return e;
    if (ev_before_field) cudaEventRecord((cudaEvent_t)ev_before_field, s);
    e = xrb::launch_field(cfg, table, nullptr, nullptr, weight_image, coords, 7, coords + 4, 7, max_samples, counters + 1, raw, 1, false, s);
    if (ev_after_field) cudaEventRecord((cudaEvent_t)ev_after_field, s);
    if (e) return e;
    return xrb_rm_calc_rgb_inference(raw, coords, numsteps, bg3_host, n_rays, rgb_act, dens_act, rgb_out, alpha_out, stream);
}

}
```

### xrnerf_b200/csrc/raymarch.cu

```cuda
#include "common.cuh"
#include <stdio.h>
#include <string.h>
#include <stdlib.h>

namespace xrb {

static thread_local char g_err[256] = "";
void set_error(const char *msg) { strncpy(g_err, msg, sizeof(g_err) - 1); g_err[sizeof(g_err) - 1] = 0; }
int check_launch(const char *what) {
    cudaError_t e = cudaGetLastError();
    if (e != cudaSuccess) { snprintf(g_err, sizeof g_err, "%s: %s", what, cudaGetErrorString(e)); return (int)e; }
    return XRB_OK;
}

constexpr uint32_t TCAP = 64;
constexpr uint32_t OVF_CAP = NERF_STEPS - TCAP;
struct OvfPool { uint32_t *counter; float *area; uint32_t n_chunks; int32_t *chunk_of; };

template <bool EMIT>
__device__ __forceinline__ uint32_t march_ray(const float o[3], const float d[3], float lo, float hi, float startt, float cone,
                                              const uint8_t *__restrict__ bitfield, uint32_t limit, float *__restrict__ coords, float *__restrict__ tbuf = nullptr,
                                              const uint32_t *lut = nullptr, const OvfPool *pool = nullptr, uint32_t ray = 0) {
    const float idir[3] = {div_(1.0f, d[0]), div_(1.0f, d[1]), div_(1.0f, d[2])};
    float wdir[3], diag = sub_(hi, lo);
    if (EMIT) { wdir[0] = mul_(add_(d[0], 1.0f), 0.5f); wdir[1] = mul_(add_(d[1], 1.0f), 0.5f); wdir[2] = mul_(add_(d[2], 1.0f), 0.5f); }
    uint32_t j = 0; float t = startt;
    float *ovf = nullptr;
    while (true) {
        float p[3] = {add_(o[0], mul_(t, d[0])), add_(o[1], mul_(t, d[1])), add_(o[2], mul_(t, d[2]))};
        if (!(aabb_contains(lo, hi, p[0], p[1], p[2]) && j < limit)) break;
        float dt = calc_dt(t, cone);
        uint32_t mip = (uint32_t)mip_from_dt(dt, p[0], p[1], p[2]);
        if (occupied_at(p[0], p[1], p[2], bitfield, mip, lut)) {
            if (EMIT) {
                float *c = coords + 7 * (size_t)j;
                c[0] = div_(sub_(p[0], lo), diag); c[1] = div_(sub_(p[1], lo), diag); c[2] = div_(sub_(p[2], lo), diag);
                c[3] = warp_dt(dt);
                c[4] = wdir[0]; c[5] = wdir[1]; c[6] = wdir[2];
            } else if (tbuf) {
                if (j < TCAP) tbuf[j] = t;
                else if (pool) {
                    if (j == TCAP) {
                        const uint32_t c = atomicAdd(pool->counter, 1u);
                        const bool got = c < pool->n_chunks;
                        pool->chunk_of[ray] = got ? (int32_t)c : -1;
                        ovf = got ? pool->area + (size_t)c * OVF_CAP : nullptr;
                    }
                    if (ovf) ovf[j - TCAP] = t;
                }
            }
            ++j; t = add_(t, dt);
        } else {
            t = advance_to_next_voxel(t, cone, p, d, idir, NERF_GRIDSIZE >> mip);
        }
    }
    return j;
}

constexpr int MARCH_BLOCK = 128;
static inline int warp_grid(int n_rays) { size_t b = ((size_t)n_rays * 32 + 255) / 256, cap = (size_t)NUM_SMS * 8; return (int)(b < cap ? (b ? b : 1) : cap); }
constexpr int MAX_LANE_STRIDE = 4;
constexpr int MARCH_RAYS_PER_BLOCK_MIN = MARCH_BLOCK / MAX_LANE_STRIDE;
static int lane_stride() { static int v = -1; if (v < 0) { const char *e = getenv("XRB_MARCH_LANE_STRIDE"); v = e ? atoi(e) : 1; if (v != 1 && v != 2 && v != 4) v = 1; } return v; }

struct MarchWs {
    uint32_t *local_excl;
    float *startt;
    uint32_t *block_sum;
    uint32_t *misc;
    float *tbuf;
    int32_t *chunk_of;
    float *ovf;
    uint32_t n_chunks;
};
__host__ __device__ inline uint32_t march_n_chunks(int n) { uint32_t c = (uint32_t)n / 8u; return c < 64u ? 64u : c; }
__host__ __device__ inline size_t march_ws_bytes(int n) {
    size_t nb = (size_t)(n + MARCH_RAYS_PER_BLOCK_MIN - 1) / MARCH_RAYS_PER_BLOCK_MIN;
    return sizeof(uint32_t) * ((size_t)n * 3 + nb + 16 + (size_t)n * TCAP + (size_t)march_n_chunks(n) * OVF_CAP);
}
inline MarchWs march_ws(void *ws, int n) {
    size_t nb = (size_t)(n + MARCH_RAYS_PER_BLOCK_MIN - 1) / MARCH_RAYS_PER_BLOCK_MIN;
    MarchWs w; w.local_excl = (uint32_t *)ws; w.startt = (float *)(w.local_excl + n); w.block_sum = (uint32_t *)(w.startt + n); w.misc = w.block_sum + nb; w.tbuf = (float *)(w.misc + 16);
    w.chunk_of = (int32_t *)(w.tbuf + (size_t)n * TCAP); w.ovf = (float *)(w.chunk_of + n); w.n_chunks = march_n_chunks(n);
    return w;
}

__device__ __forceinline__ uint32_t block_excl_scan(uint32_t v, uint32_t *total) {
    __shared__ uint32_t warp_tot[MARCH_BLOCK / 32];
    int lane = threadIdx.x & 31, w = threadIdx.x >> 5;
    uint32_t incl = warp_incl_scan_u32(v, lane);
    if (lane == 31) warp_tot[w] = incl;
    __syncthreads();
    uint32_t off = 0, tot = 0;
#pragma unroll
    for (int k = 0; k < MARCH_BLOCK / 32; ++k) { uint32_t s = warp_tot[k]; if (k < w) off += s; tot += s; }
    *total = tot;
    return off + incl - v;
}

template <int LANE_STRIDE>
__global__ void __launch_bounds__(MARCH_BLOCK) march_count_kernel(int n_rays, const float *__restrict__ rays_o, const float *__restrict__ rays_d,
                                                                  const uint8_t *__restrict__ bitfield, float lo, float hi, float near_distance, float cone,
                                                                  Pcg32 rng, uint32_t *__restrict__ local_excl, float *__restrict__ startt_out,
                                                                  uint32_t *__restrict__ block_sum, int32_t *__restrict__ numsteps, float *__restrict__ tbuf, OvfPool pool) {
    constexpr int MARCH_RAYS_PER_BLOCK = MARCH_BLOCK / LANE_STRIDE;
    __shared__ uint32_t lut[128];
    morton_lut_init(lut, threadIdx.x, MARCH_BLOCK);
    __syncthreads();
    const bool owner = (threadIdx.x % LANE_STRIDE) == 0;
    uint32_t i = blockIdx.x * MARCH_RAYS_PER_BLOCK + threadIdx.x / LANE_STRIDE;
    uint32_t n = 0;
    if (owner && i < (uint32_t)n_rays) {
        float o[3] = {rays_o[3 * (size_t)i], rays_o[3 * (size_t)i + 1], rays_o[3 * (size_t)i + 2]};
        float d[3] = {rays_d[3 * (size_t)i], rays_d[3 * (size_t)i + 1], rays_d[3 * (size_t)i + 2]};
        float st = ray_start_t(rng, i, lo, hi, o, d, near_distance, cone);
        startt_out[i] = st;
        n = march_ray<false>(o, d, lo, hi, st, cone, bitfield, NERF_STEPS, nullptr, tbuf ? tbuf + (size_t)i * TCAP : nullptr, lut, tbuf ? &pool : nullptr, i);
        numsteps[2 * (size_t)i] = (int32_t)n;
    }
    uint32_t tot;
    uint32_t ex = block_excl_scan(n, &tot);
    if (owner && i < (uint32_t)n_rays) local_excl[i] = ex;
    if (threadIdx.x == 0) block_sum[blockIdx.x] = tot;
}

__global__ void __launch_bounds__(1024) march_scan_kernel(int n_blocks, uint32_t *__restrict__ block_sum, uint32_t *__restrict__ misc, int32_t *__restrict__ counters) {
    __shared__ uint32_t warp_tot[32];
    __shared__ uint32_t carry_s;
    int lane = threadIdx.x & 31, w = threadIdx.x >> 5;
    if (threadIdx.x == 0) carry_s = 0;
    __syncthreads();
    for (int b0 = 0; b0 < n_blocks; b0 += 1024) {
        int b = b0 + threadIdx.x;
        uint32_t v = b < n_blocks ? block_sum[b] : 0u;
        uint32_t incl = warp_incl_scan_u32(v, lane);
        if (lane == 31) warp_tot[w] = incl;
        __syncthreads();
        uint32_t off = 0, tot = 0;
        for (int k = 0; k < 32; ++k) { uint32_t s = warp_tot[k]; if (k < w) off += s; tot += s; }
        uint32_t carry = carry_s;
        if (b < n_blocks) block_sum[b] = carry + off + incl - v;
        __syncthreads();
        if (threadIdx.x == 0) carry_s = carry + tot;
        __syncthreads();
    }
    if (threadIdx.x == 0) {
        uint32_t base0 = counters ? (uint32_t)counters[1] : 0u, ray0 = counters ? (uint32_t)counters[0] : 0u;
        misc[0] = base0; misc[1] = ray0; misc[2] = carry_s;
        if (counters) counters[1] = (int32_t)(base0 + carry_s);
    }
}

__global__ void __launch_bounds__(256) march_emit_kernel(int n_rays, const float *__restrict__ rays_o, const float *__restrict__ rays_d, const uint8_t *__restrict__ bitfield, float lo,
                                                         float hi, float cone, uint32_t max_samples, const uint32_t *__restrict__ local_excl, const float *__restrict__ startt,
                                                         const uint32_t *__restrict__ block_off, const uint32_t *__restrict__ misc, const float *__restrict__ tbuf,
                                                         const int32_t *__restrict__ chunk_of, const float *__restrict__ ovf, float *__restrict__ coords_out, int32_t *__restrict__ rays_index, int32_t *__restrict__ numsteps,
                                                         int32_t *__restrict__ counters, int rays_per_scan_block) {
    const int lane = threadIdx.x & 31;
    const uint32_t n_warps = (gridDim.x * 256) >> 5;
    uint32_t ok_count = 0;
    for (uint32_t i = (blockIdx.x * 256 + threadIdx.x) >> 5; i < (uint32_t)n_rays; i += n_warps) {
        uint32_t n = (uint32_t)numsteps[2 * (size_t)i];
        uint32_t base = misc[0] + block_off[i / rays_per_scan_block] + local_excl[i];
        __syncwarp();
        if (base + n > max_samples) {
            if (lane == 0) { numsteps[2 * (size_t)i] = 0; numsteps[2 * (size_t)i + 1] = (int32_t)base; }
        } else {
            ok_count += 1;
            if (lane == 0) {
                numsteps[2 * (size_t)i + 1] = (int32_t)base;
                rays_index[i] = n == 0 ? -1 : (int32_t)(misc[1] + i);
            }
            if (n > 0) {
                const float o[3] = {rays_o[3 * (size_t)i], rays_o[3 * (size_t)i + 1], rays_o[3 * (size_t)i + 2]};
                const float d[3] = {rays_d[3 * (size_t)i], rays_d[3 * (size_t)i + 1], rays_d[3 * (size_t)i + 2]};
                const float diag = sub_(hi, lo);
                const float w0 = mul_(add_(d[0], 1.0f), 0.5f), w1 = mul_(add_(d[1], 1.0f), 0.5f), w2 = mul_(add_(d[2], 1.0f), 0.5f);
                const int32_t chunk = n > TCAP ? chunk_of[i] : -1;
                const float *tl = tbuf + (size_t)i * TCAP, *to = chunk >= 0 ? ovf + (size_t)chunk * OVF_CAP : nullptr;
                const uint32_t n_par = n <= TCAP ? n : (to ? n : TCAP - 1);
                for (uint32_t j = lane; j < n_par; j += 32) {
                    float t = j < TCAP ? tl[j] : to[j - TCAP];
                    float *c = coords_out + 7 * (size_t)(base + j);
                    c[0] = div_(sub_(add_(o[0], mul_(t, d[0])), lo), diag); c[1] = div_(sub_(add_(o[1], mul_(t, d[1])), lo), diag); c[2] = div_(sub_(add_(o[2], mul_(t, d[2])), lo), diag);
                    c[3] = warp_dt(calc_dt(t, cone));
                    c[4] = w0; c[5] = w1; c[6] = w2;
                }
                if (n_par < n && lane == 0) march_ray<true>(o, d, lo, hi, tl[TCAP - 1], cone, bitfield, n - (TCAP - 1), coords_out + 7 * (size_t)(base + TCAP - 1));
            }
        }
    }
    if (lane == 0 && ok_count && counters) atomicAdd((unsigned int *)counters, ok_count);
}

__global__ void __launch_bounds__(MARCH_BLOCK) compact_count_kernel(int n_rays, const int32_t *__restrict__ numsteps, uint32_t *__restrict__ local_excl,
                                                                    uint32_t *__restrict__ block_sum) {
    uint32_t i = blockIdx.x * MARCH_BLOCK + threadIdx.x;
    uint32_t n = i < (uint32_t)n_rays ? (uint32_t)numsteps[2 * (size_t)i] : 0u;
    uint32_t tot, ex = block_excl_scan(n, &tot);
    if (i < (uint32_t)n_rays) local_excl[i] = ex;
    if (threadIdx.x == 0) block_sum[blockIdx.x] = tot;
}
__global__ void __launch_bounds__(256) compact_copy_kernel(int n_rays, uint32_t max_compacted, const float *__restrict__ coords_in, const int32_t *__restrict__ numsteps,
                                                           const uint32_t *__restrict__ local_excl, const uint32_t *__restrict__ block_off, const uint32_t *__restrict__ misc,
                                                           float *__restrict__ coords_out, int32_t *__restrict__ numsteps_c, int32_t *__restrict__ ray_counter) {
    int lane = threadIdx.x & 31;
    uint32_t ray = (blockIdx.x * 256 + threadIdx.x) >> 5;
    if (ray >= (uint32_t)n_rays) return;
    uint32_t n = (uint32_t)numsteps[2 * (size_t)ray], base = (uint32_t)numsteps[2 * (size_t)ray + 1];
    uint32_t cbase = misc[0] + block_off[ray / MARCH_BLOCK] + local_excl[ray];
    uint32_t nc = min(max_compacted - min(max_compacted, cbase), n);
    if (lane == 0) { numsteps_c[2 * (size_t)ray] = (int32_t)nc; numsteps_c[2 * (size_t)ray + 1] = (int32_t)cbase; if (nc) atomicAdd((unsigned int *)ray_counter, 1u); }
    const float *src = coords_in + 7 * (size_t)base; float *dst = coords_out + 7 * (size_t)cbase;
    for (uint32_t k = lane; k < nc * 7; k += 32) dst[k] = src[k];
}

__global__ void __launch_bounds__(256) count_trained_kernel(int n_rays, const int32_t *__restrict__ numsteps, const int32_t *__restrict__ numsteps_c, unsigned long long *__restrict__ accum) {
    unsigned int local = 0;
    for (int i = blockIdx.x * blockDim.x + threadIdx.x; i < n_rays; i += gridDim.x * blockDim.x) local += numsteps_c[2 * (size_t)i] == numsteps[2 * (size_t)i] ? 1u : 0u;
#pragma unroll
    for (int o = 16; o > 0; o >>= 1) local += __shfl_xor_sync(0xffffffffu, local, o);
    if ((threadIdx.x & 31) == 0 && local) atomicAdd(accum, (unsigned long long)local);
}

__device__ __forceinline__ float warp_excl_prod(float v, int lane, float *incl_out) {
    float incl = v;
#pragma unroll
    for (int o = 1; o < 32; o <<= 1) { float n = __shfl_up_sync(0xffffffffu, incl, o); if (lane >= o) incl *= n; }
    float ex = __shfl_up_sync(0xffffffffu, incl, 1);
    *incl_out = incl;
    return lane == 0 ? 1.f : ex;
}
__device__ __forceinline__ float warp_incl_sum(float v, int lane) {
#pragma unroll
    for (int o = 1; o < 32; o <<= 1) { float n = __shfl_up_sync(0xffffffffu, v, o); if (lane >= o) v += n; }
    return v;
}
__device__ __forceinline__ float warp_sum(float v) {
#pragma unroll
    for (int o = 16; o > 0; o >>= 1) v += __shfl_xor_sync(0xffffffffu, v, o);
    return v;
}

template <int MODE>
__global__ void __launch_bounds__(256) composite_fwd_kernel(int n_rays, const float4 *__restrict__ raw, const float *__restrict__ coords, const int32_t *__restrict__ numsteps,
                                                            const int32_t *__restrict__ numsteps_c, const float *__restrict__ bg, float3 bg_global, int rgb_act, int dens_act,
                                                            float *__restrict__ rgb_out, float *__restrict__ alpha_out) {
    int lane = threadIdx.x & 31;
    const uint32_t n_warps = (gridDim.x * 256) >> 5;
    for (uint32_t ray = (blockIdx.x * 256 + threadIdx.x) >> 5; ray < (uint32_t)n_rays; ray += n_warps) {
    const int32_t *ns = MODE == 0 ? numsteps_c : numsteps;
    uint32_t n = (uint32_t)ns[2 * (size_t)ray], base = (uint32_t)ns[2 * (size_t)ray + 1];
    float3 b = MODE == 0 ? make_float3(bg[3 * (size_t)ray], bg[3 * (size_t)ray + 1], bg[3 * (size_t)ray + 2]) : bg_global;
    if (n == 0) {
        if (lane == 0) { rgb_out[3 * (size_t)ray] = b.x; rgb_out[3 * (size_t)ray + 1] = b.y; rgb_out[3 * (size_t)ray + 2] = b.z; if (MODE == 1) alpha_out[ray] = 0.f; }
        continue;
    }
    float T = 1.f, ax = 0.f, ay = 0.f, az = 0.f;
    for (uint32_t k0 = 0; k0 < n; k0 += 32) {
        uint32_t k = k0 + lane; bool valid = k < n;
        float alpha = 0.f, cx = 0.f, cy = 0.f, cz = 0.f;
        if (valid) {
            float4 r = __ldg(raw + base + k);
            float dt = unwarp_dt(__ldg(coords + 7 * (size_t)(base + k) + 3));
            float density = net_to_density(r.w, dens_act);
            alpha = 1.f - __expf(-density * dt);
            cx = net_to_rgb(r.x, rgb_act); cy = net_to_rgb(r.y, rgb_act); cz = net_to_rgb(r.z, rgb_act);
        }
        float incl, ex = warp_excl_prod(1.f - alpha, lane, &incl);
        float w = alpha * (T * ex);
        ax += w * cx; ay += w * cy; az += w * cz;
        T *= __shfl_sync(0xffffffffu, incl, 31);
    }
    ax = warp_sum(ax); ay = warp_sum(ay); az = warp_sum(az);
    if (lane == 0) {
        bool add_bg = MODE == 1 ? true : (n == (uint32_t)numsteps[2 * (size_t)ray]);
        if (add_bg) { ax += T * b.x; ay += T * b.y; az += T * b.z; }
        rgb_out[3 * (size_t)ray] = ax; rgb_out[3 * (size_t)ray + 1] = ay; rgb_out[3 * (size_t)ray + 2] = az;
        if (MODE == 1) alpha_out[ray] = 1.f - T;
    }
    }
}

__global__ void __launch_bounds__(256) composite_bwd_kernel(int n_rays, const float4 *__restrict__ raw, const float *__restrict__ coords, const int32_t *__restrict__ numsteps_c,
                                                            const float *__restrict__ grad_rgb, const float *__restrict__ rgb_final, const float *__restrict__ grid_mean,
                                                            int rgb_act, int dens_act, float4 *__restrict__ dl_draw) {
    int lane = threadIdx.x & 31;
    const uint32_t n_warps = (gridDim.x * 256) >> 5;
    for (uint32_t ray = (blockIdx.x * 256 + threadIdx.x) >> 5; ray < (uint32_t)n_rays; ray += n_warps) {
    uint32_t n = (uint32_t)numsteps_c[2 * (size_t)ray], base = (uint32_t)numsteps_c[2 * (size_t)ray + 1];
    if (n == 0) continue;
    float loss_scale = 128.f / (float)n_rays;
    const float l2 = rgb_act == XRB_ACT_EXPONENTIAL ? 1e-4f : 0.0f;
    const float l1 = __ldg(grid_mean) < NERF_MIN_OPTICAL_THICKNESS ? 1e-4f : 0.0f;
    float gx = grad_rgb[3 * (size_t)ray], gy = grad_rgb[3 * (size_t)ray + 1], gz = grad_rgb[3 * (size_t)ray + 2];
    float fx = rgb_final[3 * (size_t)ray], fy = rgb_final[3 * (size_t)ray + 1], fz = rgb_final[3 * (size_t)ray + 2];
    float T = 1.f, px = 0.f, py = 0.f, pz = 0.f;
    for (uint32_t k0 = 0; k0 < n; k0 += 32) {
        uint32_t k = k0 + lane; bool valid = k < n;
        float4 r = make_float4(0, 0, 0, 0); float dt = 0.f, alpha = 0.f, cx = 0.f, cy = 0.f, cz = 0.f;
        if (valid) {
            r = __ldg(raw + base + k);
            dt = unwarp_dt(__ldg(coords + 7 * (size_t)(base + k) + 3));
            alpha = 1.f - __expf(-net_to_density(r.w, dens_act) * dt);
            cx = net_to_rgb(r.x, rgb_act); cy = net_to_rgb(r.y, rgb_act); cz = net_to_rgb(r.z, rgb_act);
        }
        float incl, ex = warp_excl_prod(1.f - alpha, lane, &incl);
        float Tb = T * ex, w = alpha * Tb, Ta = Tb * (1.f - alpha);
        float sx = px + warp_incl_sum(w * cx, lane), sy = py + warp_incl_sum(w * cy, lane), sz = pz + warp_incl_sum(w * cz, lane);
        if (valid) {
            float4 o;
            o.x = loss_scale * (w * gx * net_to_rgb_deriv(r.x, rgb_act) + fmaxf(0.0f, l2 * r.x));
            o.y = loss_scale * (w * gy * net_to_rgb_deriv(r.y, rgb_act) + fmaxf(0.0f, l2 * r.y));
            o.z = loss_scale * (w * gz * net_to_rgb_deriv(r.z, rgb_act) + fmaxf(0.0f, l2 * r.z));
            float dot = gx * (Ta * cx - (fx - sx)) + (gy * (Ta * cy - (fy - sy)) + gz * (Ta * cz - (fz - sz)));
            o.w = loss_scale * (net_to_density_deriv(r.w, dens_act) * (dt * dot)) + (r.w < 0.f ? -l1 : 0.0f);
            dl_draw[base + k] = o;
        }
        T *= __shfl_sync(0xffffffffu, incl, 31);
        px = __shfl_sync(0xffffffffu, sx, 31); py = __shfl_sync(0xffffffffu, sy, 31); pz = __shfl_sync(0xffffffffu, sz, 31);
    }
    }
}

constexpr int GRID_THREADS = 256;
static inline int stream_grid(size_t work_items) {
    size_t blocks = (work_items + GRID_THREADS - 1) / GRID_THREADS;
    size_t cap = (size_t)NUM_SMS * 8;
    return (int)(blocks < cap ? (blocks ? blocks : 1) : cap);
}

__global__ void __launch_bounds__(GRID_THREADS) mark_untrained_kernel(uint32_t n_elements, float *__restrict__ grid, uint32_t n_images, const float2 *__restrict__ focal,
                                                                      const float *__restrict__ xforms, int res0, int res1) {
    extern __shared__ float s_cam[];
    for (uint32_t k = threadIdx.x; k < n_images * 14; k += blockDim.x) {
        uint32_t j = k / 14, c = k % 14;
        s_cam[k] = c < 12 ? xforms[12 * (size_t)j + c] : (c == 12 ? focal[j].x : focal[j].y);
    }
    __syncthreads();
    const float half_resx = mul_((float)res0, 0.5f), half_resy = mul_((float)res1, 0.5f);
    for (uint32_t i = blockIdx.x * blockDim.x + threadIdx.x; i < n_elements; i += gridDim.x * blockDim.x) {
        uint32_t level = i / GRID_CELLS, pos_idx = i % GRID_CELLS;
        float x = (float)morton3D_invert(pos_idx >> 0), y = (float)morton3D_invert(pos_idx >> 1), z = (float)morton3D_invert(pos_idx >> 2);
        float s = __uint_as_float((127u + level) << 23);
        float px = add_(mul_(sub_(div_(add_(x, 0.5f), (float)NERF_GRIDSIZE), 0.5f), s), 0.5f);
        float py = add_(mul_(sub_(div_(add_(y, 0.5f), (float)NERF_GRIDSIZE), 0.5f), s), 0.5f);
        float pz = add_(mul_(sub_(div_(add_(z, 0.5f), (float)NERF_GRIDSIZE), 0.5f), s), 0.5f);
        float voxel_radius = div_(mul_(mul_(0.5f, SQRT3()), s), (float)NERF_GRIDSIZE);
        int count = 0;
        for (uint32_t j = 0; j < n_images; ++j) {
            const float *m = s_cam + 14 * j;
            float lx = sub_(px, m[9]), ly = sub_(py, m[10]), lz = sub_(pz, m[11]);
            float cx = add_(mul_(lx, m[0]), add_(mul_(ly, m[1]), mul_(lz, m[2])));
            float cy = add_(mul_(lx, m[3]), add_(mul_(ly, m[4]), mul_(lz, m[5])));
            float cz = add_(mul_(lx, m[6]), add_(mul_(ly, m[7]), mul_(lz, m[8])));
            if (cz > 0.f) {
                if (sub_(fabsf(cx), voxel_radius) < mul_(div_(cz, m[12]), half_resx) && sub_(fabsf(cy), voxel_radius) < mul_(div_(cz, m[13]), half_resy)) { count++; break; }
            }
        }
        grid[i] = count > 0 ? 0.f : -1.f;
    }
}

__global__ void __launch_bounds__(GRID_THREADS) generate_grid_samples_kernel(uint32_t n_elements, Pcg32 rng0, uint32_t step, float lo, float hi, const float *__restrict__ grid,
                                                                             float *__restrict__ positions, int32_t *__restrict__ indices, uint32_t n_cascades, float thresh) {
    const float diag = sub_(hi, lo);
    for (uint32_t i = blockIdx.x * blockDim.x + threadIdx.x; i < n_elements; i += gridDim.x * blockDim.x) {
        Pcg32 rng = rng0; rng.advance((uint64_t)(i * 4u));
        uint32_t level = (uint32_t)mul_(rng.next_float(), (float)n_cascades) % n_cascades;
        uint32_t idx = 0;
        for (uint32_t j = 0; j < 10; ++j) {
            idx = ((i + step * n_elements) * 56924617u + j * 19349663u + 96925573u) % GRID_CELLS;
            idx += level * GRID_CELLS;
            if (__ldg(grid + idx) > thresh) break;
        }
        uint32_t pos_idx = idx % GRID_CELLS;
        float x = (float)morton3D_invert(pos_idx >> 0), y = (float)morton3D_invert(pos_idx >> 1), z = (float)morton3D_invert(pos_idx >> 2);
        float u0 = rng.next_float(), u1 = rng.next_float(), u2 = rng.next_float();
        float s = __uint_as_float((127u + level) << 23);
        float px = add_(mul_(sub_(div_(add_(x, u0), (float)NERF_GRIDSIZE), 0.5f), s), 0.5f);
        float py = add_(mul_(sub_(div_(add_(y, u1), (float)NERF_GRIDSIZE), 0.5f), s), 0.5f);
        float pz = add_(mul_(sub_(div_(add_(z, u2), (float)NERF_GRIDSIZE), 0.5f), s), 0.5f);
        positions[3 * (size_t)i] = div_(sub_(px, lo), diag); positions[3 * (size_t)i + 1] = div_(sub_(py, lo), diag); positions[3 * (size_t)i + 2] = div_(sub_(pz, lo), diag);
        indices[i] = (int32_t)idx;
    }
}

__global__ void __launch_bounds__(GRID_THREADS) splat_kernel(uint32_t n, const int32_t *__restrict__ indices, int padded_width, const float *__restrict__ mlp_out,
                                                             float *__restrict__ grid_tmp) {
    for (uint32_t i = blockIdx.x * blockDim.x + threadIdx.x; i < n; i += gridDim.x * blockDim.x) {
        float thickness = mul_(__expf(__ldg(mlp_out + (size_t)i * padded_width)), MIN_CONE_STEPSIZE());
        atomicMax((unsigned int *)&grid_tmp[(uint32_t)indices[i]], __float_as_uint(thickness));
    }
}

__global__ void __launch_bounds__(GRID_THREADS) ema_kernel(uint32_t n4, float decay, float4 *__restrict__ grid, const float4 *__restrict__ tmp) {
    for (uint32_t i = blockIdx.x * blockDim.x + threadIdx.x; i < n4; i += gridDim.x * blockDim.x) {
        float4 g = grid[i], t = __ldg(tmp + i);
        g.x = g.x < 0.f ? g.x : fmaxf(mul_(g.x, decay), t.x); g.y = g.y < 0.f ? g.y : fmaxf(mul_(g.y, decay), t.y);
        g.z = g.z < 0.f ? g.z : fmaxf(mul_(g.z, decay), t.z); g.w = g.w < 0.f ? g.w : fmaxf(mul_(g.w, decay), t.w);
        grid[i] = g;
    }
}
__global__ void ema_tail_kernel(uint32_t start, uint32_t n, float decay, float *__restrict__ grid, const float *__restrict__ tmp) {
    uint32_t i = start + blockIdx.x * blockDim.x + threadIdx.x;
    if (i < n) { float p = grid[i]; grid[i] = p < 0.f ? p : fmaxf(mul_(p, decay), tmp[i]); }
}

constexpr int MEAN_BLOCKS = GRID_CELLS / 4096;
__global__ void __launch_bounds__(1024) grid_mean_partial_kernel(const float4 *__restrict__ grid, float *__restrict__ partial) {
    __shared__ float sdata[32];
    int lane = threadIdx.x & 31, w = threadIdx.x >> 5;
    float4 v = __ldg(grid + (size_t)blockIdx.x * 1024 + threadIdx.x);
    const float N = (float)GRID_CELLS;
    float val = add_(add_(add_(div_(fmaxf(v.x, 0.f), N), div_(fmaxf(v.y, 0.f), N)), div_(fmaxf(v.z, 0.f), N)), div_(fmaxf(v.w, 0.f), N));
#pragma unroll
    for (int o = 16; o > 0; o >>= 1) val = add_(val, __shfl_xor_sync(0xffffffffu, val, o));
    if (lane == 0) sdata[w] = val;
    __syncthreads();
    if (w == 0) {
        val = sdata[lane];
#pragma unroll
        for (int o = 16; o > 0; o >>= 1) val = add_(val, __shfl_xor_sync(0xffffffffu, val, o));
        if (lane == 0) partial[blockIdx.x] = val;
    }
}
__global__ void grid_mean_final_kernel(const float *__restrict__ partial, float *__restrict__ mean) {
    if (threadIdx.x == 0) { float t = 0.f; for (int b = 0; b < MEAN_BLOCKS; ++b) t = add_(t, partial[b]); mean[0] = t; }
}
__global__ void __launch_bounds__(GRID_THREADS) grid_to_bitfield_kernel(uint32_t n_words, const float4 *__restrict__ grid, uint32_t *__restrict__ bitfield, const float *__restrict__ mean) {
    float m = __ldg(mean);
    float thresh = NERF_MIN_OPTICAL_THICKNESS < m ? NERF_MIN_OPTICAL_THICKNESS : m;
    for (uint32_t i = blockIdx.x * blockDim.x + threadIdx.x; i < n_words; i += gridDim.x * blockDim.x) {
        uint32_t word = 0;
#pragma unroll
        for (int q = 0; q < 8; ++q) {
            float4 v = __ldg(grid + (size_t)i * 8 + q);
            uint32_t nib = (v.x > thresh ? 1u : 0u) | (v.y > thresh ? 2u : 0u) | (v.z > thresh ? 4u : 0u) | (v.w > thresh ? 8u : 0u);
            word |= nib << (4 * q);
        }
        bitfield[i] = word;
    }
}
__global__ void __launch_bounds__(GRID_THREADS) bitfield_max_pool_kernel(uint32_t n_elements, const uint2 *__restrict__ prev_level, uint8_t *__restrict__ next_level) {
    uint32_t i = blockIdx.x * blockDim.x + threadIdx.x;
    if (i >= n_elements) return;
    uint2 p = __ldg(prev_level + i);
    uint8_t bits = 0;
#pragma unroll
    for (int j = 0; j < 4; ++j) { bits |= ((p.x >> (8 * j)) & 0xffu) ? (uint8_t)(1u << j) : 0; bits |= ((p.y >> (8 * j)) & 0xffu) ? (uint8_t)(1u << (j + 4)) : 0; }
    uint32_t x = morton3D_invert(i >> 0) + NERF_GRIDSIZE / 8, y = morton3D_invert(i >> 1) + NERF_GRIDSIZE / 8, z = morton3D_invert(i >> 2) + NERF_GRIDSIZE / 8;
    next_level[morton3D(x, y, z)] |= bits;
}

}

using namespace xrb;

extern "C" {

int xrb_abi_version(void) { return 2; }
int xrb_built_for_sm(void) { return 100; }
const char *xrb_last_error(void) { return g_err; }

size_t xrb_rm_rays_sampler_workspace(int n_rays) { return march_ws_bytes(n_rays) + 2048 * sizeof(float); }

int xrb_rm_rays_sampler(const float *rays_o, const float *rays_d, const uint8_t *bitfield, const float *metadata, const int32_t *img_ids, const float *xforms,
                        int n_rays, int max_samples, float aabb0, float aabb1, float near_distance, float cone_angle, uint64_t seed, int64_t n_prior_calls,
                        float *coords_out, int32_t *rays_index, int32_t *numsteps, int32_t *counters, void *workspace, void *stream) {
    (void)metadata; (void)img_ids; (void)xforms;
    XRB_REQUIRE(n_rays >= 0 && max_samples >= 0, "rays_sampler: negative size");
    if (n_rays == 0) return XRB_OK;
    XRB_REQUIRE(rays_o && rays_d && bitfield && coords_out && rays_index && numsteps && counters && workspace, "rays_sampler: null pointer");
    cudaStream_t s = (cudaStream_t)stream;
    MarchWs w = march_ws(workspace, n_rays);
    const int ls = lane_stride(), rpb = MARCH_BLOCK / ls;
    int nb = (n_rays + rpb - 1) / rpb;
    Pcg32 rng = host_rng(seed, n_prior_calls);
    cudaMemsetAsync(w.misc + 3, 0, sizeof(uint32_t), s);
    OvfPool pool{w.misc + 3, w.ovf, w.n_chunks, w.chunk_of};
    if (ls == 1) march_count_kernel<1><<<nb, MARCH_BLOCK, 0, s>>>(n_rays, rays_o, rays_d, bitfield, aabb0, aabb1, near_distance, cone_angle, rng, w.local_excl, w.startt, w.block_sum, numsteps, w.tbuf, pool);
    else if (ls == 2) march_count_kernel<2><<<nb, MARCH_BLOCK, 0, s>>>(n_rays, rays_o, rays_d, bitfield, aabb0, aabb1, near_distance, cone_angle, rng, w.local_excl, w.startt, w.block_sum, numsteps, w.tbuf, pool);
    else march_count_kernel<4><<<nb, MARCH_BLOCK, 0, s>>>(n_rays, rays_o, rays_d, bitfield, aabb0, aabb1, near_distance, cone_angle, rng, w.local_excl, w.startt, w.block_sum, numsteps, w.tbuf, pool);
    march_scan_kernel<<<1, 1024, 0, s>>>(nb, w.block_sum, w.misc, counters);
    march_emit_kernel<<<warp_grid(n_rays), 256, 0, s>>>(n_rays, rays_o, rays_d, bitfield, aabb0, aabb1, cone_angle, (uint32_t)max_samples, w.local_excl, w.startt,
                                                                             w.block_sum, w.misc, w.tbuf, w.chunk_of, w.ovf, coords_out, rays_index, numsteps, counters, rpb);
    return check_launch("rays_sampler");
}

size_t xrb_rm_compacted_coord_workspace(int n_rays) {
    size_t nb = (size_t)(n_rays + MARCH_RAYS_PER_BLOCK_MIN - 1) / MARCH_RAYS_PER_BLOCK_MIN;
    return sizeof(uint32_t) * ((size_t)n_rays * 2 + nb + 16);
}

int xrb_rm_compacted_coord(const float *network_output, const float *coords_in, const int32_t *numsteps, int n_rays, int max_compacted, float *coords_out,
                           int32_t *numsteps_compacted, int32_t *ray_counter, int32_t *step_counter, void *workspace, void *stream) {
    (void)network_output;
    XRB_REQUIRE(n_rays >= 0 && max_compacted >= 0, "compacted_coord: negative size");
    if (n_rays == 0) return XRB_OK;
    XRB_REQUIRE(coords_in && numsteps && coords_out && numsteps_compacted && ray_counter && step_counter && workspace, "compacted_coord: null pointer");
    cudaStream_t s = (cudaStream_t)stream;
    MarchWs w = march_ws(workspace, n_rays);
    int nb = (n_rays + MARCH_BLOCK - 1) / MARCH_BLOCK;
    compact_count_kernel<<<nb, MARCH_BLOCK, 0, s>>>(n_rays, numsteps, w.local_excl, w.block_sum);
    int32_t *stage = (int32_t *)(w.misc + 4);
    cudaMemcpyAsync(stage, ray_counter, sizeof(int32_t), cudaMemcpyDeviceToDevice, s);
    cudaMemcpyAsync(stage + 1, step_counter, sizeof(int32_t), cudaMemcpyDeviceToDevice, s);
    march_scan_kernel<<<1, 1024, 0, s>>>(nb, w.block_sum, w.misc, stage);
    cudaMemcpyAsync(step_counter, stage + 1, sizeof(int32_t), cudaMemcpyDeviceToDevice, s);
    int blocks = (int)(((size_t)n_rays * 32 + 255) / 256);
    compact_copy_kernel<<<blocks, 256, 0, s>>>(n_rays, (uint32_t)max_compacted, coords_in, numsteps, w.local_excl, w.block_sum, w.misc, coords_out, numsteps_compacted, ray_counter);
    return check_launch("compacted_coord");
}

int xrb_ngp_count_trained_rays(const int32_t *numsteps, const int32_t *numsteps_compacted, int n_rays, int64_t *accum, void *stream) {
    XRB_REQUIRE(n_rays >= 0, "count_trained_rays: negative size");
    if (n_rays == 0) return XRB_OK;
    XRB_REQUIRE(numsteps && numsteps_compacted && accum && ((uintptr_t)accum & 7) == 0, "count_trained_rays: null / misaligned pointer");
    int blocks = (n_rays + 255) / 256; if (blocks > NUM_SMS * 4) blocks = NUM_SMS * 4;
    count_trained_kernel<<<blocks, 256, 0, (cudaStream_t)stream>>>(n_rays, numsteps, numsteps_compacted, (unsigned long long *)accum);
    return check_launch("count_trained_rays");
}

int xrb_rm_calc_rgb_forward(const float *raw, const float *coords, const int32_t *numsteps, const int32_t *numsteps_compacted, const float *bg, int n_rays, int rgb_act,
                            int dens_act, float *rgb_out, void *stream) {
    XRB_REQUIRE(n_rays >= 0, "calc_rgb_forward: negative size");
    if (n_rays == 0) return XRB_OK;
    XRB_REQUIRE(raw && coords && numsteps && numsteps_compacted && bg && rgb_out, "calc_rgb_forward: null pointer");
    XRB_REQUIRE(((uintptr_t)raw & 15) == 0, "calc_rgb_forward: raw must be 16-byte aligned");
    int blocks = warp_grid(n_rays);
    composite_fwd_kernel<0><<<blocks, 256, 0, (cudaStream_t)stream>>>(n_rays, (const float4 *)raw, coords, numsteps, numsteps_compacted, bg, make_float3(0, 0, 0), rgb_act, dens_act,
                                                                      rgb_out, nullptr);
    return check_launch("calc_rgb_forward");
}

int xrb_rm_calc_rgb_backward(const float *raw, const int32_t *numsteps_compacted, const float *coords, const float *grad_rgb, const float *rgb, const float *grid_mean,
                             int n_rays, int rgb_act, int dens_act, float *dl_draw, void *stream) {
    XRB_REQUIRE(n_rays >= 0, "calc_rgb_backward: negative size");
    if (n_rays == 0) return XRB_OK;
    XRB_REQUIRE(raw && coords && numsteps_compacted && grad_rgb && rgb && grid_mean && dl_draw, "calc_rgb_backward: null pointer");
    XRB_REQUIRE(((uintptr_t)raw & 15) == 0 && ((uintptr_t)dl_draw & 15) == 0, "calc_rgb_backward: raw/dl_draw must be 16-byte aligned");
    int blocks = warp_grid(n_rays);
    composite_bwd_kernel<<<blocks, 256, 0, (cudaStream_t)stream>>>(n_rays, (const float4 *)raw, coords, numsteps_compacted, grad_rgb, rgb, grid_mean, rgb_act, dens_act,
                                                                   (float4 *)dl_draw);
    return check_launch("calc_rgb_backward");
}

int xrb_rm_calc_rgb_inference(const float *raw, const float *coords, const int32_t *numsteps, const float *bg3_host, int n_rays, int rgb_act, int dens_act, float *rgb_out,
                              float *alpha_out, void *stream) {
    XRB_REQUIRE(n_rays >= 0, "calc_rgb_inference: negative size");
    if (n_rays == 0) return XRB_OK;
    XRB_REQUIRE(raw && coords && numsteps && bg3_host && rgb_out && alpha_out, "calc_rgb_inference: null pointer");
    XRB_REQUIRE(((uintptr_t)raw & 15) == 0, "calc_rgb_inference: raw must be 16-byte aligned");
    int blocks = warp_grid(n_rays);
    composite_fwd_kernel<1><<<blocks, 256, 0, (cudaStream_t)stream>>>(n_rays, (const float4 *)raw, coords, numsteps, nullptr, nullptr,
                                                                      make_float3(bg3_host[0], bg3_host[1], bg3_host[2]), rgb_act, dens_act, rgb_out, alpha_out);
    return check_launch("calc_rgb_inference");
}

int xrb_rm_mark_untrained_density_grid(const float *focal, const float *xforms, int n_elements, int n_images, int res0, int res1, float *grid, void *stream) {
    XRB_REQUIRE(n_elements >= 0 && n_images >= 0, "mark_untrained: negative size");
    if (n_elements == 0) return XRB_OK;
    XRB_REQUIRE(focal && xforms && grid, "mark_untrained: null pointer");
    size_t smem = (size_t)n_images * 14 * sizeof(float);
    XRB_REQUIRE(smem <= 200 * 1024, "mark_untrained: too many images for one shared-memory camera table (max 3657)");
    if (smem > 48 * 1024) cudaFuncSetAttribute(mark_untrained_kernel, cudaFuncAttributeMaxDynamicSharedMemorySize, (int)smem);
    mark_untrained_kernel<<<stream_grid(n_elements), GRID_THREADS, smem, (cudaStream_t)stream>>>((uint32_t)n_elements, grid, (uint32_t)n_images, (const float2 *)focal, xforms, res0, res1);
    return check_launch("mark_untrained");
}

int xrb_rm_generate_grid_samples(const float *grid, int ema_step, int n_elements, int max_cascade, float thresh, float aabb0, float aabb1, uint64_t seed, int64_t n_prior_calls,
                                 float *positions, int32_t *indices, void *stream) {
    XRB_REQUIRE(n_elements >= 0 && max_cascade >= 0 && max_cascade < (int)NERF_CASCADES, "generate_grid_samples: bad size/cascade");
    if (n_elements == 0) return XRB_OK;
    XRB_REQUIRE(grid && positions && indices, "generate_grid_samples: null pointer");
    Pcg32 rng = host_rng(seed, n_prior_calls);
    generate_grid_samples_kernel<<<stream_grid(n_elements), GRID_THREADS, 0, (cudaStream_t)stream>>>((uint32_t)n_elements, rng, (uint32_t)ema_step, aabb0, aabb1, grid, positions, indices,
                                                                                                     (uint32_t)max_cascade + 1, thresh);
    return check_launch("generate_grid_samples");
}

int xrb_rm_splat_grid_samples(const float *mlp_out, const int32_t *indices, int padded_width, int n, float *grid_tmp, void *stream) {
    XRB_REQUIRE(n >= 0 && padded_width >= 1, "splat: bad size");
    if (n == 0) return XRB_OK;
    XRB_REQUIRE(mlp_out && indices && grid_tmp, "splat: null pointer");
    splat_kernel<<<stream_grid(n), GRID_THREADS, 0, (cudaStream_t)stream>>>((uint32_t)n, indices, padded_width, mlp_out, grid_tmp);
    return check_launch("splat");
}

int xrb_rm_ema_grid_samples(const float *grid_tmp, int n_elements, float decay, float *grid, void *stream) {
    XRB_REQUIRE(n_elements >= 0, "ema: negative size");
    if (n_elements == 0) return XRB_OK;
    XRB_REQUIRE(grid_tmp && grid, "ema: null pointer");
    cudaStream_t s = (cudaStream_t)stream;
    bool aligned = (((uintptr_t)grid | (uintptr_t)grid_tmp) & 15) == 0;
    uint32_t n4 = aligned ? (uint32_t)n_elements / 4 : 0;
    if (n4) ema_kernel<<<stream_grid(n4), GRID_THREADS, 0, s>>>(n4, decay, (float4 *)grid, (const float4 *)grid_tmp);
    uint32_t rest = (uint32_t)n_elements - n4 * 4;
    if (rest) ema_tail_kernel<<<(rest + 255) / 256, 256, 0, s>>>(n4 * 4, (uint32_t)n_elements, decay, grid, grid_tmp);
    return check_launch("ema");
}

size_t xrb_rm_update_bitfield_workspace(void) { return MEAN_BLOCKS * sizeof(float); }

int xrb_rm_update_bitfield(const float *grid, float *mean, uint8_t *bitfield, void *workspace, void *stream) {
    XRB_REQUIRE(grid && mean && bitfield && workspace, "update_bitfield: null pointer");
    XRB_REQUIRE(((uintptr_t)grid & 15) == 0 && ((uintptr_t)bitfield & 7) == 0 && ((uintptr_t)workspace & 3) == 0, "update_bitfield: grid must be 16-byte, bitfield 8-byte aligned");
    cudaStream_t s = (cudaStream_t)stream;
    float *partial = (float *)workspace;
    grid_mean_partial_kernel<<<MEAN_BLOCKS, 1024, 0, s>>>((const float4 *)grid, partial);
    grid_mean_final_kernel<<<1, 32, 0, s>>>(partial, mean);
    uint32_t n_words = GRID_CELLS / 8 * NERF_CASCADES / 4;
    grid_to_bitfield_kernel<<<stream_grid(n_words), GRID_THREADS, 0, s>>>(n_words, (const float4 *)grid, (uint32_t *)bitfield, mean);
    for (uint32_t level = 1; level < NERF_CASCADES; ++level) {
        uint32_t n = GRID_CELLS / 64;
        bitfield_max_pool_kernel<<<(n + GRID_THREADS - 1) / GRID_THREADS, GRID_THREADS, 0, s>>>(n, (const uint2 *)(bitfield + (size_t)GRID_CELLS * (level - 1) / 8), bitfield + (size_t)GRID_CELLS * level / 8);
    }
    return check_launch("update_bitfield");
}

}
```

Before: 280.5 million.

## Render via compact sample records with compositing fused into field kernel

Adds a render path where the marcher emits compact (t, ray) records in place of 7-float coordinate rows. The tensor-core field kernel then rebuilds positions and directions from those records and composites in-warp with a segmented scan. Chunks at warp boundaries write partial head/tail aggregates that a small fixup kernel merges per ray. This is meant to cut the memory traffic of coordinate rows and raw outputs, and to remove the separate compositing pass, at the cost of extra complexity and per-sample ray reloads.

Result: faster. 287.4 million (median of 6 runs) (+2.5%).

```diff
diff --git a/xrnerf_b200/csrc/common.cuh b/xrnerf_b200/csrc/common.cuh
--- a/xrnerf_b200/csrc/common.cuh
+++ b/xrnerf_b200/csrc/common.cuh
@@ -172,6 +172,16 @@
     const float max_stepsize = MIN_CONE_STEPSIZE() * (1 << (NERF_CASCADES - 1));
     return add_(mul_(dt, max_stepsize - MIN_CONE_STEPSIZE()), MIN_CONE_STEPSIZE());
 }
+__device__ __forceinline__ void warped_position(const float o[3], const float d[3], float t, float lo, float diag, float p[3]) {
+#pragma unroll
+    for (int k = 0; k < 3; ++k) p[k] = div_(sub_(add_(o[k], mul_(t, d[k])), lo), diag);
+}
+__device__ __forceinline__ void warped_direction(const float d[3], float w[3]) {
+#pragma unroll
+    for (int k = 0; k < 3; ++k) w[k] = mul_(add_(d[k], 1.0f), 0.5f);
+}
+struct __align__(8) SampleRec { float t; uint32_t ray; };
+
 __device__ __forceinline__ float ray_start_t(Pcg32 rng, uint32_t i, float lo, float hi, const float o[3], const float d[3], float near_distance, float cone) {
     rng.advance((uint64_t)(i * 8u));
     float tmin = fmaxf(aabb_ray_tmin(lo, hi, o, d), near_distance);
@@ -201,6 +211,18 @@
     for (int o = 1; o < 32; o <<= 1) { uint32_t n = __shfl_up_sync(0xffffffffu, v, o); if (lane >= o) v += n; }
     return v;
 }
+__device__ __forceinline__ int warp_seg_composite(uint32_t key, int lane, float &pr, float &sx, float &sy, float &sz) {
+    const uint32_t prev_key = __shfl_up_sync(0xffffffffu, key, 1);
+    const uint32_t heads = __ballot_sync(0xffffffffu, lane == 0 || key != prev_key);
+    const int seg_start = 31 - __clz(heads & (0xffffffffu >> (31 - lane)));
+#pragma unroll
+    for (int off = 1; off < 32; off <<= 1) {
+        const float np = __shfl_up_sync(0xffffffffu, pr, off), nx = __shfl_up_sync(0xffffffffu, sx, off), ny = __shfl_up_sync(0xffffffffu, sy, off),
+                    nz = __shfl_up_sync(0xffffffffu, sz, off);
+        if (lane - off >= seg_start) { sx = nx + np * sx; sy = ny + np * sy; sz = nz + np * sz; pr = np * pr; }
+    }
+    return seg_start;
+}
 #endif
 
 }
diff --git a/xrnerf_b200/csrc/ngp_field.cuh b/xrnerf_b200/csrc/ngp_field.cuh
--- a/xrnerf_b200/csrc/ngp_field.cuh
+++ b/xrnerf_b200/csrc/ngp_field.cuh
@@ -60,6 +60,15 @@
                     const int32_t *n_dev, float *raw, cudaStream_t s);
 int launch_field(const xrb_ngp_config *cfg, const xrb_ngp_table *table, const void *dens, const void *color, const void *image, const float *pts, int pts_stride, const float *dirs,
                  int dirs_stride, int n, const int32_t *n_dev, float *out, int impl, bool density_only, cudaStream_t s);
+
+struct RecComposite {
+    const SampleRec *recs; const float *rays_o, *rays_d;
+    float lo, hi, cone, bg0, bg1, bg2; int rgb_act, dens_act;
+    float *rgb_out, *alpha_out; float4 *head, *tail;
+};
+int launch_field_records(const xrb_ngp_config *cfg, const xrb_ngp_table *table, const void *image, int n, const int32_t *n_dev, const RecComposite &rc, cudaStream_t s);
+int march_records(const float *rays_o, const float *rays_d, const uint8_t *bitfield, int n_rays, int max_samples, float aabb0, float aabb1, float near_distance, float cone_angle,
+                  uint64_t seed, int64_t n_prior_calls, SampleRec *recs_out, int32_t *numsteps, int32_t *counters, void *workspace, const int32_t **n_rows_dev, cudaStream_t s);
 
 #ifdef __CUDACC__
 __device__ __forceinline__ float round_h(float x) { return __half2float(__float2half_rn(x)); }
diff --git a/xrnerf_b200/csrc/ngp_fused.cu b/xrnerf_b200/csrc/ngp_fused.cu
--- a/xrnerf_b200/csrc/ngp_fused.cu
+++ b/xrnerf_b200/csrc/ngp_fused.cu
@@ -275,22 +275,22 @@
                             if (cand < 32 && b <= q) j = cand;
                         }
                         const uint32_t bj = __shfl_sync(0xffffffffu, rbase, j);
-                        float x = 0.5f, y = 0.5f, z = 0.5f, wd0 = 0.5f, wd1 = 0.5f, wd2 = 0.5f;
+                        float p[3] = {0.5f, 0.5f, 0.5f}, wd[3] = {0.5f, 0.5f, 0.5f};
                         if (valid) {
                             const float tt = *(volatile float *)(tb + (size_t)j * FR_TCAP + (q - bj));
                             const size_t rj = (size_t)grp * 32 + j;
-                            const float oj0 = __ldg(P.rays_o + 3 * rj), oj1 = __ldg(P.rays_o + 3 * rj + 1), oj2 = __ldg(P.rays_o + 3 * rj + 2);
-                            const float dj0 = __ldg(P.rays_d + 3 * rj), dj1 = __ldg(P.rays_d + 3 * rj + 1), dj2 = __ldg(P.rays_d + 3 * rj + 2);
-                            x = div_(sub_(add_(oj0, mul_(tt, dj0)), P.lo), diag); y = div_(sub_(add_(oj1, mul_(tt, dj1)), P.lo), diag); z = div_(sub_(add_(oj2, mul_(tt, dj2)), P.lo), diag);
-                            wd0 = mul_(add_(dj0, 1.0f), 0.5f); wd1 = mul_(add_(dj1, 1.0f), 0.5f); wd2 = mul_(add_(dj2, 1.0f), 0.5f);
+                            const float oj[3] = {__ldg(P.rays_o + 3 * rj), __ldg(P.rays_o + 3 * rj + 1), __ldg(P.rays_o + 3 * rj + 2)};
+                            const float dj[3] = {__ldg(P.rays_d + 3 * rj), __ldg(P.rays_d + 3 * rj + 1), __ldg(P.rays_d + 3 * rj + 2)};
+                            warped_position(oj, dj, tt, P.lo, diag, p);
+                            warped_direction(dj, wd);
                             dtc = unwarp_dt(warp_dt(calc_dt(tt, P.cone)));
                             key = j;
                         }
 #ifdef XRB_FUSED_TIMERS
-                        if (P.dbg & 8) { if (__float_as_uint(x + y + z + dtc) == 0x7fc12345u) pc[6] += 1; }
+                        if (P.dbg & 8) { if (__float_as_uint(p[0] + p[1] + p[2] + dtc) == 0x7fc12345u) pc[6] += 1; }
 #endif
                         PTICK(1);
-                        submit_chunk(x, y, z, wd0, wd1, wd2);
+                        submit_chunk(p[0], p[1], p[2], wd[0], wd[1], wd[2]);
                         PTICK(2);
                     }
                     if (pending) {
@@ -306,15 +306,7 @@
                             sx = alpha * net_to_rgb(raw.x, P.rgb_act); sy = alpha * net_to_rgb(raw.y, P.rgb_act); sz = alpha * net_to_rgb(raw.z, P.rgb_act);
                         }
                         float pr = 1.f - alpha;
-                        const uint32_t prev_key = __shfl_up_sync(0xffffffffu, pend_key, 1);
-                        const uint32_t heads = __ballot_sync(0xffffffffu, lane == 0 || pend_key != prev_key);
-                        const int seg_start = 31 - __clz(heads & (0xffffffffu >> (31 - lane)));
-#pragma unroll
-                        for (int off = 1; off < 32; off <<= 1) {
-                            const float np = __shfl_up_sync(0xffffffffu, pr, off), nx = __shfl_up_sync(0xffffffffu, sx, off), ny = __shfl_up_sync(0xffffffffu, sy, off),
-                                        nz = __shfl_up_sync(0xffffffffu, sz, off);
-                            if ((int)lane - off >= seg_start) { sx = nx + np * sx; sy = ny + np * sy; sz = nz + np * sz; pr = np * pr; }
-                        }
+                        warp_seg_composite(pend_key, (int)lane, pr, sx, sy, sz);
                         const uint32_t pq0 = q0 - 32;
                         const uint32_t lo_q = max(rbase, pq0), hi_q = min(rbase + m, q0);
                         const uint32_t tail = (hi_q - 1 - pq0) & 31;
diff --git a/xrnerf_b200/csrc/ngp_mlp.cu b/xrnerf_b200/csrc/ngp_mlp.cu
--- a/xrnerf_b200/csrc/ngp_mlp.cu
+++ b/xrnerf_b200/csrc/ngp_mlp.cu
@@ -143,22 +143,83 @@
     }
 }
 
-template <bool DENSITY_ONLY, int NWG, int MAXREG, int NP>
+constexpr uint32_t NO_RAY = 0xffffffffu;
+__device__ __forceinline__ SampleRec rec_fetch(const RecComposite &rc, int i, int n) { return i < n ? rc.recs[i] : SampleRec{0.f, NO_RAY}; }
+__device__ __forceinline__ void rec_inputs(const RecComposite &rc, const SampleRec &r, float &x, float &y, float &z, float &dx, float &dy, float &dz) {
+    if (r.ray == NO_RAY) return;
+    const float o[3] = {__ldg(rc.rays_o + 3 * (size_t)r.ray), __ldg(rc.rays_o + 3 * (size_t)r.ray + 1), __ldg(rc.rays_o + 3 * (size_t)r.ray + 2)};
+    const float d[3] = {__ldg(rc.rays_d + 3 * (size_t)r.ray), __ldg(rc.rays_d + 3 * (size_t)r.ray + 1), __ldg(rc.rays_d + 3 * (size_t)r.ray + 2)};
+    float p[3], w[3];
+    warped_position(o, d, r.t, rc.lo, sub_(rc.hi, rc.lo), p);
+    warped_direction(d, w);
+    x = p[0]; y = p[1]; z = p[2]; dx = w[0]; dy = w[1]; dz = w[2];
+}
+__device__ __forceinline__ uint32_t rec_neighbour(const RecComposite &rc, int i, int n, int lane) {
+    if (lane == 0 && i > 0 && i <= n) return rc.recs[i - 1].ray;
+    if (lane == 31 && i + 1 < n) return rc.recs[i + 1].ray;
+    return NO_RAY;
+}
+__device__ __forceinline__ void rec_composite(const RecComposite &rc, int i, int lane, float4 raw, float t, uint32_t key, uint32_t nb) {
+    float alpha = 0.f, sx = 0.f, sy = 0.f, sz = 0.f;
+    if (key != NO_RAY) {
+        alpha = 1.f - __expf(-net_to_density(raw.w, rc.dens_act) * unwarp_dt(warp_dt(calc_dt(t, rc.cone))));
+        sx = alpha * net_to_rgb(raw.x, rc.rgb_act); sy = alpha * net_to_rgb(raw.y, rc.rgb_act); sz = alpha * net_to_rgb(raw.z, rc.rgb_act);
+    }
+    float pr = 1.f - alpha;
+    const int seg_start = warp_seg_composite(key, lane, pr, sx, sy, sz);
+    const uint32_t next_key = __shfl_down_sync(0xffffffffu, key, 1), before = __shfl_sync(0xffffffffu, nb, 0), after = __shfl_sync(0xffffffffu, nb, 31);
+    if (key == NO_RAY || (lane != 31 && next_key == key)) return;
+    const bool from_prev = seg_start == 0 && before == key, into_next = lane == 31 && after == key;
+    if (!from_prev && !into_next) {
+        rc.rgb_out[3 * (size_t)key] = sx + pr * rc.bg0; rc.rgb_out[3 * (size_t)key + 1] = sy + pr * rc.bg1; rc.rgb_out[3 * (size_t)key + 2] = sz + pr * rc.bg2;
+        rc.alpha_out[key] = 1.f - pr;
+        return;
+    }
+    const float4 agg = make_float4(pr, sx, sy, sz);
+    if (from_prev) rc.head[i >> 5] = agg;
+    if (into_next) rc.tail[i >> 5] = agg;
+}
+template <bool DENSITY_ONLY, int NWG, int MAXREG, int NP, bool REC>
 __global__ void __launch_bounds__(128 * NWG, NWG == 2 ? 2 : 1) __maxnreg__(MAXREG)
 ngp_field_tc_kernel(HashGridDev g, const __half2 *__restrict__ table, const uint8_t *__restrict__ cells, const void *__restrict__ weight_image, uint32_t image_bytes, int density_hidden,
                     int color_hidden, const float *__restrict__ pts, int pts_stride, const float *__restrict__ dirs, int dirs_stride, int n, const int32_t *__restrict__ n_dev,
-                    float *__restrict__ out, int dbg) {
+                    float *__restrict__ out, int dbg, const __grid_constant__ RecComposite rc) {
     extern __shared__ uint8_t dyn_smem[];
     if (n_dev) n = min(n, max(*n_dev, 0));
+    const int lane = threadIdx.x & 31;
     constexpr uint32_t TMEM_COLS = NWG <= 2 ? 128 : (NWG <= 4 ? 256 : 512);
     TcWarpgroup c = tc_cta_setup<NWG, TMEM_COLS>(dyn_smem, weight_image, image_bytes);
     const uint32_t tmem_base = c.tmem - c.wg * 64;
     const WeightImageLayout L = weight_image_layout(density_hidden, color_hidden);
     const int n_tiles = (n + 127) / 128;
-    if (!(dbg & 7)) {
+    if (REC || !(dbg & 7)) {
         const int stride = gridDim.x * NWG;
         int tile = blockIdx.x * NWG + c.wg;
-        if (tile < n_tiles) {
+        if (REC && tile < n_tiles) {
+            uint32_t e[16];
+            float dx = 0.5f, dy = 0.5f, dz = 0.5f;
+            {
+                float x = 0.5f, y = 0.5f, z = 0.5f;
+                rec_inputs(rc, rec_fetch(rc, tile * 128 + c.row, n), x, y, z, dx, dy, dz);
+                tc_gather_levels<NP, 0, 16>(table, cells, g, x, y, z, e);
+            }
+            SampleRec rn = rec_fetch(rc, tile + stride < n_tiles ? (tile + stride) * 128 + c.row : n, n);
+            for (; tile < n_tiles; tile += stride) {
+                const int i = tile * 128 + c.row;
+                const bool has_next = tile + stride < n_tiles;
+                float xn = 0.5f, yn = 0.5f, zn = 0.5f, dxn = 0.5f, dyn = 0.5f, dzn = 0.5f;
+                if (has_next) rec_inputs(rc, rn, xn, yn, zn, dxn, dyn, dzn);
+                rn = rec_fetch(rc, tile + 2 * stride < n_tiles ? i + 2 * stride * 128 : n, n);
+                const SampleRec cur = rec_fetch(rc, i, n);
+                const uint32_t nb = rec_neighbour(rc, i, n, lane);
+                uint32_t en[16];
+                const float4 raw = tc_field_gather_ahead<NP, false>(c, L, density_hidden, color_hidden, table, cells, g, e, dx, dy, dz, has_next, xn, yn, zn, en);
+                rec_composite(rc, i, lane, raw, cur.t, cur.ray, nb);
+#pragma unroll
+                for (int k = 0; k < 16; ++k) e[k] = en[k];
+                dx = dxn; dy = dyn; dz = dzn;
+            }
+        } else if (!REC && tile < n_tiles) {
             uint32_t e[16];
             float dx = 0.5f, dy = 0.5f, dz = 0.5f;
             {
@@ -363,13 +424,15 @@
         const int npl = tab->n_packed_levels;
         const int np = (plan_valid(g, npl) && (npl == 6 || npl == 7)) ? npl : 0;
         int n_tiles = (n + 127) / 128;
+        const RecComposite no_rc{};
 #define XRB_LAUNCH_TC(D, NWG, R, NP)                                                                                                                \
     do {                                                                                                                                            \
-        auto k = ngp_field_tc_kernel<D, NWG, R, NP>;                                                                                                \
+        auto k = ngp_field_tc_kernel<D, NWG, R, NP, false>;                                                                                         \
         const size_t smem = tc_cta_smem_bytes<NWG>(image_bytes);                                                                                    \
         cudaFuncSetAttribute(k, cudaFuncAttributeMaxDynamicSharedMemorySize, (int)smem);                                                            \
         int grid = persistent_grid((const void *)k, 128 * NWG, smem, (n_tiles + NWG - 1) / NWG, NWG == 2 ? 2 : 1);                                  \
-        k<<<grid, 128 * NWG, smem, s>>>(g, (const __half2 *)table, cells, image, image_bytes, cfg->density_hidden, cfg->color_hidden, pts, pts_stride, dirs, dirs_stride, n, n_dev, out, dbg); \
+        k<<<grid, 128 * NWG, smem, s>>>(g, (const __half2 *)table, cells, image, image_bytes, cfg->density_hidden, cfg->color_hidden, pts, pts_stride, dirs, dirs_stride, n, n_dev, out, dbg, \
+                                        no_rc);                                                                                                     \
     } while (0)
 #define XRB_LAUNCH_TC_NP(D, NWG, R)                                                                                                                 \
     do {                                                                                                                                            \
@@ -386,6 +449,21 @@
     }
     return check_launch(density_only ? "ngp_density_forward" : "ngp_mlp_forward");
 }
+
+int launch_field_records(const xrb_ngp_config *cfg, const xrb_ngp_table *tab, const void *image, int n, const int32_t *n_dev, const RecComposite &rc, cudaStream_t s) {
+    HashGridDev g; int e = table_setup(cfg, tab, &g, "field"); if (e) return e;
+    const uint32_t image_bytes = weight_image_layout(cfg->density_hidden, cfg->color_hidden).total;
+    const int npl = tab->n_packed_levels;
+    const int np = (plan_valid(g, npl) && (npl == 6 || npl == 7)) ? npl : 0;
+    const int n_tiles = (n + 127) / 128;
+    auto k = np == 6 ? ngp_field_tc_kernel<false, 2, 96, 6, true> : (np == 7 ? ngp_field_tc_kernel<false, 2, 96, 7, true> : ngp_field_tc_kernel<false, 2, 96, 0, true>);
+    const size_t smem = tc_cta_smem_bytes<2>(image_bytes);
+    cudaFuncSetAttribute(k, cudaFuncAttributeMaxDynamicSharedMemorySize, (int)smem);
+    const int grid = persistent_grid((const void *)k, 256, smem, (n_tiles + 1) / 2, 2);
+    k<<<grid, 256, smem, s>>>(g, (const __half2 *)tab->table_fp16, (const uint8_t *)tab->cell_image, image, image_bytes, cfg->density_hidden, cfg->color_hidden, nullptr, 3, nullptr, 3,
+                              n, n_dev, nullptr, 0, rc);
+    return check_launch("ngp_field (records)");
+}
 }
 extern "C" {
 
diff --git a/xrnerf_b200/csrc/ngp_render.cu b/xrnerf_b200/csrc/ngp_render.cu
--- a/xrnerf_b200/csrc/ngp_render.cu
+++ b/xrnerf_b200/csrc/ngp_render.cu
@@ -1,34 +1,67 @@
 #include "ngp_field.cuh"
+
+namespace xrb {
+
+__global__ void __launch_bounds__(256) composite_fixup_kernel(int n_rays, const int32_t *__restrict__ numsteps, const float4 *__restrict__ head, const float4 *__restrict__ tail,
+                                                              float3 bg, float *__restrict__ rgb_out, float *__restrict__ alpha_out) {
+    const uint32_t ray = blockIdx.x * blockDim.x + threadIdx.x;
+    if (ray >= (uint32_t)n_rays) return;
+    const uint32_t n = (uint32_t)numsteps[2 * (size_t)ray], base = (uint32_t)numsteps[2 * (size_t)ray + 1];
+    float P = 1.f, sx = 0.f, sy = 0.f, sz = 0.f;
+    if (n > 0) {
+        const uint32_t c0 = base >> 5, c1 = (base + n - 1) >> 5;
+        if (c0 == c1) return;
+        const float4 a = tail[c0];
+        P = a.x; sx = a.y; sy = a.z; sz = a.w;
+        for (uint32_t c = c0 + 1; c <= c1; ++c) {
+            const float4 h = head[c];
+            sx += P * h.y; sy += P * h.z; sz += P * h.w; P *= h.x;
+        }
+    }
+    rgb_out[3 * (size_t)ray] = sx + P * bg.x; rgb_out[3 * (size_t)ray + 1] = sy + P * bg.y; rgb_out[3 * (size_t)ray + 2] = sz + P * bg.z;
+    alpha_out[ray] = 1.f - P;
+}
+
+static size_t march_part(int n_rays) { return (xrb_rm_rays_sampler_workspace(n_rays) + 255) & ~(size_t)255; }
+static size_t n_row_chunks(int max_samples) { return ((size_t)max_samples + 31) / 32; }
+
+}
+
+using namespace xrb;
 
 extern "C" {
 
 size_t xrb_ngp_render_workspace(int n_rays, int max_samples) {
-    size_t a = (xrb_rm_rays_sampler_workspace(n_rays) + 255) & ~(size_t)255;
-    return a + (size_t)max_samples * (7 + 4) * sizeof(float) + (size_t)n_rays * sizeof(int32_t) + 256;
+    return march_part(n_rays) + 2 * n_row_chunks(max_samples) * sizeof(float4) + (size_t)max_samples * sizeof(SampleRec) + 256;
 }
 
 int xrb_ngp_render(const xrb_ngp_config *cfg, const xrb_ngp_table *table, const void *weight_image, const uint8_t *bitfield, const float *rays_o, const float *rays_d, int n_rays,
                    int max_samples, float aabb0, float aabb1, float near_distance, float cone_angle, uint64_t seed, int64_t n_prior_calls, const float *bg3_host, int rgb_act,
                    int dens_act, float *rgb_out, float *alpha_out, int32_t *numsteps, int32_t *counters, void *workspace, void *ev_before_field, void *ev_after_field, void *stream) {
-    int e = xrb::check_cfg(cfg); if (e) return e;
+    int e = check_cfg(cfg); if (e) return e;
     XRB_REQUIRE(n_rays >= 0 && max_samples > 0, "ngp_render: bad size");
     if (n_rays == 0) return XRB_OK;
     XRB_REQUIRE(table && weight_image && bitfield && rays_o && rays_d && bg3_host && rgb_out && alpha_out && numsteps && counters && workspace, "ngp_render: null pointer");
+    XRB_REQUIRE(((uintptr_t)workspace & 15) == 0, "ngp_render: workspace must be 16-byte aligned");
     cudaStream_t s = (cudaStream_t)stream;
     uint8_t *ws = (uint8_t *)workspace;
-    size_t a = (xrb_rm_rays_sampler_workspace(n_rays) + 255) & ~(size_t)255;
-    float *coords = (float *)(ws + a);
-    float *raw = coords + (size_t)max_samples * 7;
-    int32_t *rays_index = (int32_t *)(raw + (size_t)max_samples * 4);
+    const size_t nc = n_row_chunks(max_samples);
+    float4 *head = (float4 *)(ws + march_part(n_rays)), *tail = head + nc;
+    SampleRec *recs = (SampleRec *)(tail + nc);
     cudaMemsetAsync(counters, 0, 2 * sizeof(int32_t), s);
-    e = xrb_rm_rays_sampler(rays_o, rays_d, bitfield, nullptr, nullptr, nullptr, n_rays, max_samples, aabb0, aabb1, near_distance, cone_angle, seed, n_prior_calls, coords, rays_index,
-                            numsteps, counters, ws, stream);
+    const int32_t *n_rows = nullptr;
+    e = march_records(rays_o, rays_d, bitfield, n_rays, max_samples, aabb0, aabb1, near_distance, cone_angle, seed, n_prior_calls, recs, numsteps, counters, ws, &n_rows, s);
     if (e) return e;
     if (ev_before_field) cudaEventRecord((cudaEvent_t)ev_before_field, s);
-    e = xrb::launch_field(cfg, table, nullptr, nullptr, weight_image, coords, 7, coords + 4, 7, max_samples, counters + 1, raw, 1, false, s);
+    RecComposite rc;
+    rc.recs = recs; rc.rays_o = rays_o; rc.rays_d = rays_d;
+    rc.lo = aabb0; rc.hi = aabb1; rc.cone = cone_angle; rc.bg0 = bg3_host[0]; rc.bg1 = bg3_host[1]; rc.bg2 = bg3_host[2]; rc.rgb_act = rgb_act; rc.dens_act = dens_act;
+    rc.rgb_out = rgb_out; rc.alpha_out = alpha_out; rc.head = head; rc.tail = tail;
+    e = launch_field_records(cfg, table, weight_image, max_samples, n_rows, rc, s);
+    if (e) return e;
+    composite_fixup_kernel<<<(n_rays + 255) / 256, 256, 0, s>>>(n_rays, numsteps, head, tail, make_float3(bg3_host[0], bg3_host[1], bg3_host[2]), rgb_out, alpha_out);
     if (ev_after_field) cudaEventRecord((cudaEvent_t)ev_after_field, s);
-    if (e) return e;
-    return xrb_rm_calc_rgb_inference(raw, coords, numsteps, bg3_host, n_rays, rgb_act, dens_act, rgb_out, alpha_out, stream);
+    return check_launch("ngp_render");
 }
 
 }
diff --git a/xrnerf_b200/csrc/raymarch.cu b/xrnerf_b200/csrc/raymarch.cu
--- a/xrnerf_b200/csrc/raymarch.cu
+++ b/xrnerf_b200/csrc/raymarch.cu
@@ -17,13 +17,14 @@
 constexpr uint32_t OVF_CAP = NERF_STEPS - TCAP;
 struct OvfPool { uint32_t *counter; float *area; uint32_t n_chunks; int32_t *chunk_of; };
 
-template <bool EMIT>
+enum { EMIT_ROWS = 1, EMIT_RECS = 2 };
+template <int EMIT>
 __device__ __forceinline__ uint32_t march_ray(const float o[3], const float d[3], float lo, float hi, float startt, float cone,
                                               const uint8_t *__restrict__ bitfield, uint32_t limit, float *__restrict__ coords, float *__restrict__ tbuf = nullptr,
-                                              const uint32_t *lut = nullptr, const OvfPool *pool = nullptr, uint32_t ray = 0) {
+                                              const uint32_t *lut = nullptr, const OvfPool *pool = nullptr, uint32_t ray = 0, SampleRec *__restrict__ recs = nullptr) {
     const float idir[3] = {div_(1.0f, d[0]), div_(1.0f, d[1]), div_(1.0f, d[2])};
     float wdir[3], diag = sub_(hi, lo);
-    if (EMIT) { wdir[0] = mul_(add_(d[0], 1.0f), 0.5f); wdir[1] = mul_(add_(d[1], 1.0f), 0.5f); wdir[2] = mul_(add_(d[2], 1.0f), 0.5f); }
+    if (EMIT == EMIT_ROWS) warped_direction(d, wdir);
     uint32_t j = 0; float t = startt;
     float *ovf = nullptr;
     while (true) {
@@ -32,7 +33,9 @@
         float dt = calc_dt(t, cone);
         uint32_t mip = (uint32_t)mip_from_dt(dt, p[0], p[1], p[2]);
         if (occupied_at(p[0], p[1], p[2], bitfield, mip, lut)) {
-            if (EMIT) {
+            if (EMIT == EMIT_RECS) {
+                recs[j] = SampleRec{t, ray};
+            } else if (EMIT == EMIT_ROWS) {
                 float *c = coords + 7 * (size_t)j;
                 c[0] = div_(sub_(p[0], lo), diag); c[1] = div_(sub_(p[1], lo), diag); c[2] = div_(sub_(p[2], lo), diag);
                 c[3] = warp_dt(dt);
@@ -57,6 +60,7 @@
     return j;
 }
 
+constexpr int MISC_ROWS_END = 6;
 constexpr int MARCH_BLOCK = 128;
 static inline int warp_grid(int n_rays) { size_t b = ((size_t)n_rays * 32 + 255) / 256, cap = (size_t)NUM_SMS * 8; return (int)(b < cap ? (b ? b : 1) : cap); }
 constexpr int MAX_LANE_STRIDE = 4;
@@ -115,7 +119,7 @@
         float d[3] = {rays_d[3 * (size_t)i], rays_d[3 * (size_t)i + 1], rays_d[3 * (size_t)i + 2]};
         float st = ray_start_t(rng, i, lo, hi, o, d, near_distance, cone);
         startt_out[i] = st;
-        n = march_ray<false>(o, d, lo, hi, st, cone, bitfield, NERF_STEPS, nullptr, tbuf ? tbuf + (size_t)i * TCAP : nullptr, lut, tbuf ? &pool : nullptr, i);
+        n = march_ray<0>(o, d, lo, hi, st, cone, bitfield, NERF_STEPS, nullptr, tbuf ? tbuf + (size_t)i * TCAP : nullptr, lut, tbuf ? &pool : nullptr, i);
         numsteps[2 * (size_t)i] = (int32_t)n;
     }
     uint32_t tot;
@@ -146,50 +150,64 @@
     }
     if (threadIdx.x == 0) {
         uint32_t base0 = counters ? (uint32_t)counters[1] : 0u, ray0 = counters ? (uint32_t)counters[0] : 0u;
-        misc[0] = base0; misc[1] = ray0; misc[2] = carry_s;
+        misc[0] = base0; misc[1] = ray0; misc[2] = carry_s; misc[MISC_ROWS_END] = base0 + carry_s;
         if (counters) counters[1] = (int32_t)(base0 + carry_s);
     }
 }
 
+template <bool REC>
 __global__ void __launch_bounds__(256) march_emit_kernel(int n_rays, const float *__restrict__ rays_o, const float *__restrict__ rays_d, const uint8_t *__restrict__ bitfield, float lo,
                                                          float hi, float cone, uint32_t max_samples, const uint32_t *__restrict__ local_excl, const float *__restrict__ startt,
-                                                         const uint32_t *__restrict__ block_off, const uint32_t *__restrict__ misc, const float *__restrict__ tbuf,
-                                                         const int32_t *__restrict__ chunk_of, const float *__restrict__ ovf, float *__restrict__ coords_out, int32_t *__restrict__ rays_index, int32_t *__restrict__ numsteps,
-                                                         int32_t *__restrict__ counters, int rays_per_scan_block) {
-    const int lane = threadIdx.x & 31;
-    const uint32_t n_warps = (gridDim.x * 256) >> 5;
+                                                         const uint32_t *__restrict__ block_off, uint32_t *__restrict__ misc, const float *__restrict__ tbuf,
+                                                         const int32_t *__restrict__ chunk_of, const float *__restrict__ ovf, float *__restrict__ coords_out, SampleRec *__restrict__ recs_out,
+                                                         int32_t *__restrict__ rays_index, int32_t *__restrict__ numsteps, int32_t *__restrict__ counters, int rays_per_scan_block) {
+    constexpr int G = REC ? 8 : 32;
+    const int lane = threadIdx.x & 31, gl = lane % G;
+    const uint32_t gmask = G == 32 ? 0xffffffffu : ((1u << G) - 1u) << (lane - gl);
+    const uint32_t n_groups = (gridDim.x * 256) / G;
     uint32_t ok_count = 0;
-    for (uint32_t i = (blockIdx.x * 256 + threadIdx.x) >> 5; i < (uint32_t)n_rays; i += n_warps) {
+    for (uint32_t i = (blockIdx.x * 256 + threadIdx.x) / G; i < (uint32_t)n_rays; i += n_groups) {
         uint32_t n = (uint32_t)numsteps[2 * (size_t)i];
         uint32_t base = misc[0] + block_off[i / rays_per_scan_block] + local_excl[i];
-        __syncwarp();
+        __syncwarp(gmask);
         if (base + n > max_samples) {
-            if (lane == 0) { numsteps[2 * (size_t)i] = 0; numsteps[2 * (size_t)i + 1] = (int32_t)base; }
+            if (gl == 0) { numsteps[2 * (size_t)i] = 0; numsteps[2 * (size_t)i + 1] = (int32_t)base; atomicMin(misc + MISC_ROWS_END, base); }
         } else {
-            ok_count += 1;
-            if (lane == 0) {
+            ok_count += gl == 0;
+            if (gl == 0) {
                 numsteps[2 * (size_t)i + 1] = (int32_t)base;
-                rays_index[i] = n == 0 ? -1 : (int32_t)(misc[1] + i);
+                if (!REC) rays_index[i] = n == 0 ? -1 : (int32_t)(misc[1] + i);
             }
             if (n > 0) {
-                const float o[3] = {rays_o[3 * (size_t)i], rays_o[3 * (size_t)i + 1], rays_o[3 * (size_t)i + 2]};
-                const float d[3] = {rays_d[3 * (size_t)i], rays_d[3 * (size_t)i + 1], rays_d[3 * (size_t)i + 2]};
-                const float diag = sub_(hi, lo);
-                const float w0 = mul_(add_(d[0], 1.0f), 0.5f), w1 = mul_(add_(d[1], 1.0f), 0.5f), w2 = mul_(add_(d[2], 1.0f), 0.5f);
                 const int32_t chunk = n > TCAP ? chunk_of[i] : -1;
                 const float *tl = tbuf + (size_t)i * TCAP, *to = chunk >= 0 ? ovf + (size_t)chunk * OVF_CAP : nullptr;
                 const uint32_t n_par = n <= TCAP ? n : (to ? n : TCAP - 1);
-                for (uint32_t j = lane; j < n_par; j += 32) {
-                    float t = j < TCAP ? tl[j] : to[j - TCAP];
-                    float *c = coords_out + 7 * (size_t)(base + j);
-                    c[0] = div_(sub_(add_(o[0], mul_(t, d[0])), lo), diag); c[1] = div_(sub_(add_(o[1], mul_(t, d[1])), lo), diag); c[2] = div_(sub_(add_(o[2], mul_(t, d[2])), lo), diag);
-                    c[3] = warp_dt(calc_dt(t, cone));
-                    c[4] = w0; c[5] = w1; c[6] = w2;
+                if (REC) {
+                    for (uint32_t j = gl; j < n_par; j += G) recs_out[base + j] = SampleRec{j < TCAP ? tl[j] : to[j - TCAP], i};
+                } else {
+                    const float o[3] = {rays_o[3 * (size_t)i], rays_o[3 * (size_t)i + 1], rays_o[3 * (size_t)i + 2]};
+                    const float d[3] = {rays_d[3 * (size_t)i], rays_d[3 * (size_t)i + 1], rays_d[3 * (size_t)i + 2]};
+                    const float diag = sub_(hi, lo);
+                    float w[3]; warped_direction(d, w);
+                    for (uint32_t j = gl; j < n_par; j += G) {
+                        float t = j < TCAP ? tl[j] : to[j - TCAP];
+                        float *c = coords_out + 7 * (size_t)(base + j);
+                        float p[3]; warped_position(o, d, t, lo, diag, p);
+                        c[0] = p[0]; c[1] = p[1]; c[2] = p[2];
+                        c[3] = warp_dt(calc_dt(t, cone));
+                        c[4] = w[0]; c[5] = w[1]; c[6] = w[2];
+                    }
                 }
-                if (n_par < n && lane == 0) march_ray<true>(o, d, lo, hi, tl[TCAP - 1], cone, bitfield, n - (TCAP - 1), coords_out + 7 * (size_t)(base + TCAP - 1));
+                if (n_par < n && gl == 0) {
+                    const float o[3] = {rays_o[3 * (size_t)i], rays_o[3 * (size_t)i + 1], rays_o[3 * (size_t)i + 2]};
+                    const float d[3] = {rays_d[3 * (size_t)i], rays_d[3 * (size_t)i + 1], rays_d[3 * (size_t)i + 2]};
+                    if (REC) march_ray<EMIT_RECS>(o, d, lo, hi, tl[TCAP - 1], cone, bitfield, n - (TCAP - 1), nullptr, nullptr, nullptr, nullptr, i, recs_out + base + TCAP - 1);
+                    else march_ray<EMIT_ROWS>(o, d, lo, hi, tl[TCAP - 1], cone, bitfield, n - (TCAP - 1), coords_out + 7 * (size_t)(base + TCAP - 1));
+                }
             }
         }
     }
+    ok_count = __reduce_add_sync(0xffffffffu, ok_count);
     if (lane == 0 && ok_count && counters) atomicAdd((unsigned int *)counters, ok_count);
 }
 
@@ -465,15 +483,11 @@
 
 size_t xrb_rm_rays_sampler_workspace(int n_rays) { return march_ws_bytes(n_rays) + 2048 * sizeof(float); }
 
-int xrb_rm_rays_sampler(const float *rays_o, const float *rays_d, const uint8_t *bitfield, const float *metadata, const int32_t *img_ids, const float *xforms,
-                        int n_rays, int max_samples, float aabb0, float aabb1, float near_distance, float cone_angle, uint64_t seed, int64_t n_prior_calls,
-                        float *coords_out, int32_t *rays_index, int32_t *numsteps, int32_t *counters, void *workspace, void *stream) {
-    (void)metadata; (void)img_ids; (void)xforms;
-    XRB_REQUIRE(n_rays >= 0 && max_samples >= 0, "rays_sampler: negative size");
-    if (n_rays == 0) return XRB_OK;
-    XRB_REQUIRE(rays_o && rays_d && bitfield && coords_out && rays_index && numsteps && counters && workspace, "rays_sampler: null pointer");
-    cudaStream_t s = (cudaStream_t)stream;
-    MarchWs w = march_ws(workspace, n_rays);
+}
+namespace xrb {
+static void launch_march(const float *rays_o, const float *rays_d, const uint8_t *bitfield, int n_rays, int max_samples, float aabb0, float aabb1, float near_distance,
+                         float cone_angle, uint64_t seed, int64_t n_prior_calls, float *coords_out, SampleRec *recs_out, int32_t *rays_index, int32_t *numsteps, int32_t *counters,
+                         const MarchWs &w, cudaStream_t s) {
     const int ls = lane_stride(), rpb = MARCH_BLOCK / ls;
     int nb = (n_rays + rpb - 1) / rpb;
     Pcg32 rng = host_rng(seed, n_prior_calls);
@@ -483,8 +497,33 @@
     else if (ls == 2) march_count_kernel<2><<<nb, MARCH_BLOCK, 0, s>>>(n_rays, rays_o, rays_d, bitfield, aabb0, aabb1, near_distance, cone_angle, rng, w.local_excl, w.startt, w.block_sum, numsteps, w.tbuf, pool);
     else march_count_kernel<4><<<nb, MARCH_BLOCK, 0, s>>>(n_rays, rays_o, rays_d, bitfield, aabb0, aabb1, near_distance, cone_angle, rng, w.local_excl, w.startt, w.block_sum, numsteps, w.tbuf, pool);
     march_scan_kernel<<<1, 1024, 0, s>>>(nb, w.block_sum, w.misc, counters);
-    march_emit_kernel<<<warp_grid(n_rays), 256, 0, s>>>(n_rays, rays_o, rays_d, bitfield, aabb0, aabb1, cone_angle, (uint32_t)max_samples, w.local_excl, w.startt,
-                                                                             w.block_sum, w.misc, w.tbuf, w.chunk_of, w.ovf, coords_out, rays_index, numsteps, counters, rpb);
+    if (recs_out)
+        march_emit_kernel<true><<<warp_grid(n_rays), 256, 0, s>>>(n_rays, rays_o, rays_d, bitfield, aabb0, aabb1, cone_angle, (uint32_t)max_samples, w.local_excl, w.startt,
+                                                                  w.block_sum, w.misc, w.tbuf, w.chunk_of, w.ovf, nullptr, recs_out, nullptr, numsteps, counters, rpb);
+    else
+        march_emit_kernel<false><<<warp_grid(n_rays), 256, 0, s>>>(n_rays, rays_o, rays_d, bitfield, aabb0, aabb1, cone_angle, (uint32_t)max_samples, w.local_excl, w.startt,
+                                                                   w.block_sum, w.misc, w.tbuf, w.chunk_of, w.ovf, coords_out, nullptr, rays_index, numsteps, counters, rpb);
+}
+
+int march_records(const float *rays_o, const float *rays_d, const uint8_t *bitfield, int n_rays, int max_samples, float aabb0, float aabb1, float near_distance, float cone_angle,
+                  uint64_t seed, int64_t n_prior_calls, SampleRec *recs_out, int32_t *numsteps, int32_t *counters, void *workspace, const int32_t **n_rows_dev, cudaStream_t s) {
+    MarchWs w = march_ws(workspace, n_rays);
+    launch_march(rays_o, rays_d, bitfield, n_rays, max_samples, aabb0, aabb1, near_distance, cone_angle, seed, n_prior_calls, nullptr, recs_out, nullptr, numsteps, counters, w, s);
+    *n_rows_dev = (const int32_t *)(w.misc + MISC_ROWS_END);
+    return check_launch("march_records");
+}
+}
+extern "C" {
+
+int xrb_rm_rays_sampler(const float *rays_o, const float *rays_d, const uint8_t *bitfield, const float *metadata, const int32_t *img_ids, const float *xforms,
+                        int n_rays, int max_samples, float aabb0, float aabb1, float near_distance, float cone_angle, uint64_t seed, int64_t n_prior_calls,
+                        float *coords_out, int32_t *rays_index, int32_t *numsteps, int32_t *counters, void *workspace, void *stream) {
+    (void)metadata; (void)img_ids; (void)xforms;
+    XRB_REQUIRE(n_rays >= 0 && max_samples >= 0, "rays_sampler: negative size");
+    if (n_rays == 0) return XRB_OK;
+    XRB_REQUIRE(rays_o && rays_d && bitfield && coords_out && rays_index && numsteps && counters && workspace, "rays_sampler: null pointer");
+    launch_march(rays_o, rays_d, bitfield, n_rays, max_samples, aabb0, aabb1, near_distance, cone_angle, seed, n_prior_calls, coords_out, nullptr, rays_index, numsteps, counters,
+                 march_ws(workspace, n_rays), (cudaStream_t)stream);
     return check_launch("rays_sampler");
 }
 
```
